# Sinica-SLAM/vae_npvc

Measured on AMD Instinct MI355X. Metric: mel-frames/sec/GPU VQ-VAE train step (80-dim mel, batch=64x256f) at 1/2/4/8 GPUs, higher is better.
Workload: dtype bf16; 1 GPU; vcc20 VQ-VAE (K=512, 80-mel), 64x256 frames per GPU; global_batch=64, seq_len=256, parallelism=dp1

## Files before the change

include/vqx.h:

```cpp
#ifndef VQX_H
#define VQX_H

#include <stdint.h>

#ifdef __cplusplus
extern "C" {
#endif

typedef void* vqx_stream_t;

enum { VQX_F32 = 0, VQX_BF16 = 1 };

enum {
  VQX_PRO_NONE = 0,
  VQX_PRO_LRELU = 1,
  VQX_PRO_RELU = 2,
  VQX_PRO_SCALE_RELU = 3
};

enum {
  VQX_EPI_BIAS = 1 << 0,
  VQX_EPI_ROWBIAS = 1 << 1,
  VQX_EPI_MASK = 1 << 2,
  VQX_EPI_RES = 1 << 3,
  VQX_EPI_GNADD = 1 << 4,
  VQX_EPI_SPLIT = 1 << 5,
  VQX_EPI_OUTF32 = 1 << 6,
  VQX_EPI_ACT = 1 << 7,
  VQX_EPI_ACT2 = 1 << 8,
  VQX_EPI_COLSUM = 1 << 9,
  VQX_EPI_GNSTATS = 1 << 10,
  VQX_EPI_GNBWD = 1 << 11
};
#define VQX_CONV_TILE_ROWS 128

typedef struct vqx_conv_args {
  const void* x;
  const void* w;
  void* y;
  const float* bias;
  const float* rowbias;
  const void* res;
  const void* mask;
  const void* gn_h;
  const float* gn_mean_rstd;
  const float* gn_gamma;
  const float* gn_beta;
  float* out2;
  int64_t n_rows;
  int32_t T;
  int32_t cin, cout, ntaps, pad;
  int32_t ldx, ldy, ldres, ldmask, ldgn, ldo2;
  int32_t dtype;
  int32_t prologue;
  int32_t epilogue;
  int32_t split_col, out2_accumulate;
  float pro_scale, mask_slope, mask_scale;
  void* y2;
  int32_t ldy2, epi_act;
  float* colsum_part;
  float* stat_part;
  int32_t gn_groups, gn_glu;
  const float* gn_stat_tiles;
  float gn_eps;
  int32_t dil;
  int32_t kernel_policy;
  int32_t rowbias_T;
} vqx_conv_args;

#define VQX_POLICY_AUTO 0
#define VQX_POLICY_IM2COL 1
#define VQX_POLICY_TALL256 2
#define VQX_POLICY_TALL512 3
#define VQX_POLICY_TR128 4
#define VQX_POLICY_K1_2PCU 5

int vqx_conv1d_fwd(const vqx_conv_args* a, vqx_stream_t stream);
int vqx_conv1d_dgrad(const vqx_conv_args* a, vqx_stream_t stream);

typedef struct vqx_wgrad_args {
  const void* p;
  const void* q;
  void* slabs;
  int64_t n_rows;
  int32_t T, r_dim, c_dim, ntaps, pad, shift_sign, ldp, ldq;
  int32_t dtype, q_prologue, splits;
  float pro_scale;
  int32_t dil;
  int32_t slab_dtype;
  int32_t kernel_policy;
  float* fixup_dw;
  uint32_t* fixup_counters;
} vqx_wgrad_args;

int vqx_conv1d_wgrad(const vqx_wgrad_args* a, vqx_stream_t stream);
int vqx_wgrad_fixup_ok(int64_t n_rows, int32_t T, int32_t r_dim, int32_t c_dim, int32_t ntaps, int32_t pad, int32_t dil,
                       int32_t dtype, int32_t slab_dtype, int32_t q_prologue, int32_t policy, int32_t* ok);

int vqx_conv1d_dgrad_wgrad(const vqx_conv_args* d, const vqx_wgrad_args* w, int32_t* fused, vqx_stream_t stream);

#define VQX_WN_COLREDUCE 2
#define VQX_WN_RESAMPLE 3
#define VQX_WN_RESAMPLE_T 4
typedef struct vqx_wn_layer {
  const float* v;
  const float* g;
  void* w_packed;
  float* norm;
  float* dv;
  float* dg;
  const void* slabs;
  int32_t kind, cout, cin, k, splits, dtype;
  int32_t stride, pad;
  int32_t slab_dtype;
} vqx_wn_layer;

int vqx_weight_norm_fwd(const vqx_wn_layer* layers_host, const vqx_wn_layer* layers_dev,
                        int32_t n_layers, vqx_stream_t stream);
#define VQX_WNF_NORMS_READY 1
int vqx_weight_norm_fwd_flags(const vqx_wn_layer* layers_host, const vqx_wn_layer* layers_dev,
                              int32_t n_layers, int32_t flags, vqx_stream_t stream);
int vqx_weight_norm_bwd(const vqx_wn_layer* layers_host, const vqx_wn_layer* layers_dev,
                        int32_t n_layers, vqx_stream_t stream);
int vqx_weight_norm_bwd_partials(const vqx_wn_layer* layers_host, int32_t n_layers, int64_t* count);
int vqx_weight_norm_bwd_sq(const vqx_wn_layer* layers_host, const vqx_wn_layer* layers_dev,
                           int32_t n_layers, float* sq_partials, int64_t sq_capacity, vqx_stream_t stream);
int vqx_sq_norm_finish(const float* partials, int64_t n_partials, const float* g, const int64_t* ranges,
                       int32_t n_ranges, float* scratch , float* out, vqx_stream_t stream);
int vqx_sq_norm_finish_adam(const float* partials, int64_t n_partials, const float* g, const int64_t* ranges,
                            int32_t n_ranges, float* scratch, float* out, int64_t* step, double lr0, double gamma,
                            int32_t step_size, double beta1, double beta2, double eps, float* hyper,
                            vqx_stream_t stream);

int vqx_groupnorm_stats(const void* x, int32_t ldx, int32_t dtype, int64_t n_rows, int32_t T,
                        int32_t C, int32_t G, float eps, float* partials ,
                        float* mean_rstd, vqx_stream_t stream);

int vqx_gn_glu_fwd(const void* u, int32_t ldu, void* g, int32_t ldg, int32_t dtype, int64_t n_rows,
                   int32_t T, int32_t C, const float* mean_rstd, const float* gamma, const float* beta,
                   vqx_stream_t stream);

int vqx_gn_glu_fwd_tiles(const void* u, int32_t ldu, void* g, int32_t ldg, int32_t dtype, int64_t n_rows,
                         int32_t T, int32_t C, const float* parts, float eps, float* mean_rstd,
                         const float* gamma, const float* beta, vqx_stream_t stream);

int vqx_gn_lrelu_fwd(const void* h, int32_t ldh, void* g, int32_t ldg, int32_t dtype, int64_t n_rows, int32_t T,
                     int32_t C, const float* mean_rstd, const float* gamma, const float* beta, vqx_stream_t stream);

int vqx_gn_bwd(const void* dy, int32_t lddy, const void* u, int32_t ldu, void* du, int32_t lddu,
               int32_t dtype, int64_t n_rows, int32_t T, int32_t C, int32_t G, int32_t glu,
               const float* mean_rstd, const float* gamma, const float* beta,
               float* partials ,
               int32_t nparts ,
               float* colsum_b , float* dgamma_b , float* dbeta_b ,
               vqx_stream_t stream);

int vqx_gn_finalize_tiles(const float* parts, int64_t n_rows, int32_t T, int32_t C, int32_t G, float eps,
                          float* mean_rstd, vqx_stream_t stream);

int vqx_colsum(const void* x, int32_t ldx, int32_t dtype, int64_t n_rows, int32_t C,
               float* partials , float* out, int32_t accumulate, vqx_stream_t stream);

int vqx_colsum_parts(int64_t n_rows, int32_t C, int32_t dtype, int32_t* nparts);
int vqx_colsum_partials(const void* x, int32_t ldx, int32_t dtype, int64_t n_rows, int32_t C,
                        float* partials , vqx_stream_t stream);

int vqx_nct_to_ntc(const float* x_nct, int32_t B, int32_t C, int32_t T, void* y, int32_t ldy,
                   int32_t dtype, vqx_stream_t stream);
int vqx_ntc_to_nct(const void* y, int32_t ldy, int32_t dtype, int32_t B, int32_t C, int32_t T,
                   float* x_nct, vqx_stream_t stream);

int vqx_logloss_fwd_bwd(const float* x_nct, const float* xhat, int32_t ldxh, int32_t B, int32_t C,
                        int32_t T, float grad_scale, void* dxhat, int32_t lddx, int32_t dtype,
                        float* loss_out, float* partials, vqx_stream_t stream);
int vqx_logloss_fwd_bwd_x(const float* x, const float* xhat, int32_t ldxh, int32_t B, int32_t C, int32_t T,
                          float grad_scale, void* dxhat, int32_t lddx, int32_t dtype, float* loss_out,
                          float* partials, const float* extra_partials, int32_t n_extra, float* extra_out,
                          vqx_stream_t stream);
int vqx_logloss_parts(const float* x, const float* xhat, int32_t ldxh, int32_t B, int32_t C, int32_t T,
                      float grad_scale, void* dxhat, int32_t lddx, int32_t dtype, float* partials, int32_t* n_parts,
                      vqx_stream_t stream);

int vqx_vq_forward(const float* z, int64_t n_rows, int32_t D, const float* E, int32_t K,
                   int64_t* idx, float* zq, void* zq_c, int32_t zq_c_dtype, float* sqerr_out,
                   float* partials, float* bsum, float* bcnt, vqx_stream_t stream);
int vqx_vq_workspace(int64_t n_rows, int32_t K, int32_t D, int32_t with_stats, int64_t* floats);
int vqx_vq_stats(const float* z, int64_t n_rows, int32_t D, const int64_t* idx, int32_t K, float* partials,
                 float* bsum, float* bcnt, vqx_stream_t stream);

int vqx_vq_ema_update(float* emb_sum, float* emb_elem, float* E, const float* bsum,
                      const float* bcnt, const float* rand_rows, int32_t K, int32_t D, float mu,
                      float threshold, float* diag, float* partials, vqx_stream_t stream);
int vqx_vq_ema_update_clear(float* emb_sum, float* emb_elem, float* E, float* bsum, float* bcnt,
                            const float* rand_rows, int32_t K, int32_t D, float mu, float threshold, float* diag,
                            float* partials, vqx_stream_t stream);
typedef struct {
  const float* parts[2];
  int32_t n[2];
  float scale[2];
  float* out[2];
  const float* pub_src;
  int32_t pub_n;
  float* pub_copy;
  void* pub_box;
  int32_t pub_slot, pub_slots, pub_floats;
  uint32_t pub_seq;
  const float* rows_src;
  int32_t rows_ld, n_rows;
  const int32_t* rows_host;
} vqx_step_close;
int vqx_vq_ema_update_close(float* emb_sum, float* emb_elem, float* E, float* bsum, float* bcnt,
                            const float* rand_rows, int32_t K, int32_t D, float mu, float threshold, float* diag,
                            float* partials, const vqx_step_close* close, vqx_stream_t stream);

int vqx_gather_rows(const float* src, int32_t ld_src, const int64_t* rows, int32_t n_out,
                    int32_t D, float* out, vqx_stream_t stream);

int vqx_gather_rows_host(const float* src, int32_t ld_src, const int32_t* rows, int32_t n_out,
                         int32_t D, float* out, vqx_stream_t stream);

int vqx_vq_commit_bwd(const float* z, const float* zq, int64_t count, float scale, void* dz,
                      int32_t dtype, vqx_stream_t stream);
#define VQX_COMMIT_PARTS 256
int vqx_vq_commit_bwd_cs(const float* z, const float* zq, int64_t n_rows, int32_t D, float scale, void* dz,
                         int32_t dtype, float* partials , vqx_stream_t stream);

int vqx_time_gather(const void* x, void* y, int32_t B, int32_t T, int32_t C, const int32_t* src_t,
                    int32_t dtype, vqx_stream_t stream);

int vqx_crop_batch(const float* corpus, int64_t n_rows, int32_t mel, const int64_t* spk_table, int32_t n_utts,
                   const int64_t* row0, const int32_t* len, const int32_t* utt, int32_t B, int32_t T, float* x,
                   int64_t* y, vqx_stream_t stream);

int vqx_embedding_fwd(const float* weight, const int64_t* ids, int32_t B, int32_t D, float* out,
                      vqx_stream_t stream);
int vqx_embedding_bwd(const float* dout, const int64_t* ids, int32_t B, int32_t D, float* dweight,
                      vqx_stream_t stream);
int vqx_embedding_bwd_rows(const float* dout, const int64_t* ids, int32_t B, int32_t D, int32_t n_rows,
                           float* dweight, int32_t accumulate, vqx_stream_t stream);

typedef struct vqx_linear_layer {
  const float* W;
  const float* bias;
  float* out;
  const float* dout;
// ... 10 lines not shown
                      const vqx_linear_layer* cond_table_dev, int32_t n_cond, const float* emb,
                      const int64_t* ids, int32_t B, int32_t I, int32_t O, const float* x_nct, int32_t xB,
                      int32_t C, int32_t T, void* y, int32_t ldy, int32_t y_dtype, vqx_stream_t stream);
int vqx_linear_batched_bwd_ids(const vqx_linear_layer* table_dev, int32_t n, const float* emb,
                               const int64_t* ids, int32_t B, int32_t I, int32_t O, float* dc, float* partials,
                               vqx_stream_t stream);

int vqx_linear_f32(const float* c, const float* W, const float* bias, int32_t B, int32_t I,
                   int32_t O, float* out, vqx_stream_t stream);
int vqx_linear_bwd_f32(const float* dout, const float* c, const float* W, int32_t B, int32_t I,
                       int32_t O, float* dW, float* dc, vqx_stream_t stream);

int vqx_grad_sq_norm(const float* g, int64_t n, float* partials, float* out, vqx_stream_t stream);
int vqx_adam_hyper(int64_t* step, double lr0, double gamma, int32_t step_size, double beta1,
                   double beta2, double eps, float* hyper, vqx_stream_t stream);
int vqx_adam_step(float* p, const float* g, float* m, float* v, int64_t n, const float* hyper,
                  const float* sumsq, float max_norm, vqx_stream_t stream);
int vqx_adam_step_wn(float* p, const float* g, float* m, float* v, int64_t n, const float* hyper,
                     const float* sumsq, float max_norm, const vqx_wn_layer* rows_host,
                     const vqx_wn_layer* rows_dev, int32_t n_layers, const int64_t* segs_host,
                     const int64_t* segs_dev, int32_t n_segs, vqx_stream_t stream);

int vqx_radam_hyper(int64_t* step, double lr0, double gamma, int32_t step_size, double beta1,
                    double beta2, double eps, float* hyper, vqx_stream_t stream);
int vqx_radam_step(float* p, const float* g, float* m, float* v, int64_t n, const float* hyper,
                   const float* sumsq, float max_norm, vqx_stream_t stream);

#define VQX_MULTI_MAX_TENSORS 128
#define VQX_MULTI_CHUNK 4096
int vqx_multi_chunks(const int64_t* numel, int32_t n, int64_t* out);
int vqx_multi_sq_norm(const float* const* grads, const int64_t* numel, int32_t n, float* partials,
                      int64_t n_partials, vqx_stream_t stream);
int vqx_multi_adam_step(float* p, float* m, float* v, int64_t n_flat, const int64_t* offset,
                        const int64_t* numel, const float* const* grads, int32_t n, const float* hyper,
                        const float* sumsq, float max_norm, int32_t kind, vqx_stream_t stream);

int vqx_vq_normalize(const float* z, int64_t n_rows, int32_t D, float* E, int32_t K, float* z_norm,
                     float* z_len, float* emb_norm, float* e_len, float* partials, float* normloss_out,
                     vqx_stream_t stream);
int vqx_vq_perplexity(const float* counts, int32_t K, int64_t n_rows, float* out, vqx_stream_t stream);
int vqx_vq_plain_bwd(const float* z, const float* z_norm, const float* z_len, const float* zq,
                     const void* dzq, const int32_t* src_t, int32_t T, int64_t n_rows, int32_t D,
                     int32_t normalize, float beta, float scale, void* dz, int32_t dtype, const float* bsum,
                     const float* bcnt, const float* emb, const float* e_len, int32_t K, float* dE,
                     vqx_stream_t stream);

int vqx_vq_plain_bwd_g(const float* z, const float* z_norm, const float* z_len, const float* zq, const void* dzq,
                       int32_t T, int64_t n_rows, int32_t D, int32_t normalize, float s_qut, float s_enc,
                       const float* g_qut, const float* g_enc, void* dz, int32_t dtype, const float* bsum,
                       const float* bcnt, const float* emb, const float* e_len, int32_t K, float* dE,
                       vqx_stream_t stream);

int vqx_scale_act_2d(const void* src, int32_t ld_src, int32_t src_dtype, void* dst, int32_t ld_dst,
                     int32_t dst_dtype, int64_t rows, int32_t cols, float scale, int32_t act,
                     vqx_stream_t stream);

int vqx_convert_2d(const void* src, int32_t ld_src, int32_t src_dtype, void* dst, int32_t ld_dst,
                   int32_t dst_dtype, int64_t rows, int32_t cols, vqx_stream_t stream);
int vqx_convert_2d_zero2(const void* src, int32_t ld_src, int32_t src_dtype, void* dst, int32_t ld_dst,
                         int32_t dst_dtype, int64_t rows, int32_t cols, void* zero_dst, int32_t ld_zero,
                         int64_t zero_rows, int32_t zero_cols, vqx_stream_t stream);

int vqx_wgrad_tiles(int64_t n_rows, int32_t T, int32_t r_dim, int32_t c_dim, int32_t ntaps, int32_t pad,
                    int32_t dil, int32_t dtype, int32_t q_prologue, int32_t kernel_policy ,
                    int32_t* tiles);

const char* vqx_last_error(void);

int vqx_probe_enable(int32_t on);
int vqx_probe_select(const int32_t* info5);
int vqx_probe_clear(void);
int vqx_probe_count(int64_t* n);
int vqx_probe_read(int64_t i, int32_t* info5, double* flops, float* ms);

int vqx_stream_create_cu_mask(int32_t reserve_cus, vqx_stream_t* out, int32_t* cus_used);
int vqx_stream_destroy(vqx_stream_t stream);

int vqx_mailbox_create(int32_t slots, int32_t floats, void** host, void** dev);
int vqx_mailbox_destroy(void* host);
int vqx_mailbox_publish(const float* src, int32_t n, float* dev_copy, void* box_dev, int32_t slot, int32_t slots,
                        int32_t floats, uint32_t seq, vqx_stream_t stream);

typedef struct {
  const float* z;
  const float* gst_embs;
  const float *wq, *bq, *wk, *bk, *wv, *bv, *wo, *bo;
  float* style;
  float* ws;
  const float* d_style;
  float* dz;
  float* d_gst_embs;
  float *dwq, *dbq, *dwk, *dbk, *dwv, *dbv, *dwo, *dbo;
  int32_t B, T, R, N, E, F, H, ldz, lddz;
} vqx_gst_args;
int vqx_gst_workspace(int32_t B, int32_t N, int32_t F, int32_t H, int32_t R, int32_t E, int64_t* floats);
int vqx_gst_fwd(const vqx_gst_args* a, vqx_stream_t stream);
int vqx_gst_bwd(const vqx_gst_args* a, vqx_stream_t stream);

typedef struct vqx_hier_level {
  void* z;
  int32_t T_l, C, ld;
} vqx_hier_level;
int vqx_upsample_cat_fwd(const vqx_hier_level* levels, int32_t n_levels, int32_t B, int32_t T, void* out,
                         int32_t ldo, int32_t out_dtype, vqx_stream_t stream);
int vqx_upsample_cat_bwd(const vqx_hier_level* levels, int32_t n_levels, int32_t B, int32_t T, const void* dout,
                         int32_t ldo, int32_t dout_dtype, vqx_stream_t stream);
int vqx_upsample_cat_bwd_to(const vqx_hier_level* levels, int32_t n_levels, int32_t B, int32_t T, const void* dout,
                            int32_t ldo, int32_t dout_dtype, int32_t level_dtype, vqx_stream_t stream);

typedef struct vqx_codes_level {
  const void* z;
  const int64_t* idx;
  int32_t T_l, C, ld;
  int32_t K, normalize;
} vqx_codes_level;
int vqx_codes_upsample_cat(const vqx_codes_level* levels, int32_t n_levels, int32_t B, int32_t T, void* out,
                           int32_t ldo, int32_t out_dtype, vqx_stream_t stream);

int vqx_nct_to_ntc_lrelu_bwd(const float* g_nct, int32_t B, int32_t C, int32_t T, const void* a, int32_t lda,
                             int32_t a_dtype, float slope, void* dst, int32_t lddst, int32_t dst_dtype,
                             vqx_stream_t stream);

int vqx_ntc_to_nct_scale(const float* y, int32_t ldy, int32_t B, int32_t C, int32_t T, const float* g,
                         float* x_nct, vqx_stream_t stream);

int vqx_ntc_to_nct_gather(const void* y, int32_t ldy, int32_t dtype, int32_t B, int32_t C, int32_t T,
                          const int32_t* src_t, float* x_nct, vqx_stream_t stream);
int vqx_nct_to_ntc_keep(const float* g_nct, int32_t B, int32_t C, int32_t T, const int32_t* src_t, void* y,
                        int32_t ldy, int32_t dtype, vqx_stream_t stream);
int vqx_vq_commit_bwd_g(const float* z, const float* zq, int32_t B, int32_t D, int32_t T, float s, const float* g,
                        int32_t nct, float* dz, vqx_stream_t stream);

int vqx_groupnorm_stats_len(const void* x, int32_t ldx, int32_t dtype, int64_t n_rows, int32_t T, int32_t C,
                            int32_t G, const int32_t* len, float eps, float* partials, float* mean_rstd,
                            vqx_stream_t stream);
int vqx_gn_lrelu_fwd_len(const void* h, int32_t ldh, void* g, int32_t ldg, int32_t dtype, int64_t n_rows, int32_t T,
                         int32_t C, const int32_t* len, const float* mean_rstd, const float* gamma, const float* beta,
                         vqx_stream_t stream);
int vqx_gn_glu_fwd_len(const void* u, int32_t ldu, void* g, int32_t ldg, int32_t dtype, int64_t n_rows, int32_t T,
                       int32_t C, const int32_t* len, const float* mean_rstd, const float* gamma, const float* beta,
                       vqx_stream_t stream);
int vqx_mask_tail(void* x, int32_t ldx, int32_t dtype, int64_t n_rows, int32_t T, int32_t C, const int32_t* len,
                  vqx_stream_t stream);
int vqx_codes_upsample_cat_len(const vqx_codes_level* levels, int32_t n_levels, int32_t B, int32_t T,
                               const int32_t* n_len, const int32_t* m_len, void* out, int32_t ldo, int32_t out_dtype,
                               vqx_stream_t stream);
int vqx_segment_mean(const float* z, int32_t ldz, int64_t n_rows, int32_t T, int32_t C, const int32_t* len,
                     float* out, int32_t ldo, vqx_stream_t stream);
int vqx_nct_to_ntc_len(const float* x_nct, int32_t B, int32_t C, int32_t T, const int32_t* len, void* y, int32_t ldy,
                       int32_t dtype, vqx_stream_t stream);
int vqx_ntc_to_nct_len(const void* y, int32_t ldy, int32_t dtype, int32_t B, int32_t C, int32_t T, const int32_t* len,
                       float* x_nct, int32_t T_out, vqx_stream_t stream);

#define VQX_ABI_VERSION 130
int vqx_version(void);

#ifdef __cplusplus
}
#endif
#endif
```

vae_npvc_amd/_lib.py:

```python
import ctypes
import os
from pathlib import Path

import torch

LIB_PATH = Path(__file__).resolve().parent / "lib" / "libvqx.so"
ABI_VERSION = 130

VQX_F32, VQX_BF16 = 0, 1
PRO_NONE, PRO_LRELU, PRO_RELU, PRO_SCALE_RELU = 0, 1, 2, 3
(EPI_BIAS, EPI_ROWBIAS, EPI_MASK, EPI_RES, EPI_GNADD, EPI_SPLIT, EPI_OUTF32, EPI_ACT, EPI_ACT2, EPI_COLSUM, EPI_GNSTATS,
 EPI_GNBWD) = (1 << i for i in range(12))
CONV_TILE_ROWS = 128

c_void_p, c_int32, c_int64, c_float, c_double = (ctypes.c_void_p, ctypes.c_int32, ctypes.c_int64,
                                                 ctypes.c_float, ctypes.c_double)


class ConvArgs(ctypes.Structure):
    _fields_ = [
        ("x", c_void_p), ("w", c_void_p), ("y", c_void_p), ("bias", c_void_p), ("rowbias", c_void_p),
        ("res", c_void_p), ("mask", c_void_p), ("gn_h", c_void_p), ("gn_mean_rstd", c_void_p),
        ("gn_gamma", c_void_p), ("gn_beta", c_void_p), ("out2", c_void_p),
        ("n_rows", c_int64), ("T", c_int32), ("cin", c_int32), ("cout", c_int32), ("ntaps", c_int32),
        ("pad", c_int32), ("ldx", c_int32), ("ldy", c_int32), ("ldres", c_int32), ("ldmask", c_int32),
        ("ldgn", c_int32), ("ldo2", c_int32), ("dtype", c_int32), ("prologue", c_int32),
        ("epilogue", c_int32), ("split_col", c_int32), ("out2_accumulate", c_int32),
        ("pro_scale", c_float), ("mask_slope", c_float), ("mask_scale", c_float),
        ("y2", c_void_p), ("ldy2", c_int32), ("epi_act", c_int32), ("colsum_part", c_void_p),
        ("stat_part", c_void_p), ("gn_groups", c_int32), ("gn_glu", c_int32),
        ("gn_stat_tiles", c_void_p), ("gn_eps", c_float), ("dil", c_int32), ("kernel_policy", c_int32),
        ("rowbias_T", c_int32),
    ]


class WgradArgs(ctypes.Structure):
    _fields_ = [
        ("p", c_void_p), ("q", c_void_p), ("slabs", c_void_p), ("n_rows", c_int64), ("T", c_int32),
        ("r_dim", c_int32), ("c_dim", c_int32), ("ntaps", c_int32), ("pad", c_int32),
        ("shift_sign", c_int32), ("ldp", c_int32), ("ldq", c_int32), ("dtype", c_int32),
        ("q_prologue", c_int32), ("splits", c_int32), ("pro_scale", c_float), ("dil", c_int32),
        ("slab_dtype", c_int32), ("kernel_policy", c_int32), ("fixup_dw", c_void_p), ("fixup_counters", c_void_p),
    ]


class WNLayer(ctypes.Structure):
    _fields_ = [
        ("v", c_void_p), ("g", c_void_p), ("w_packed", c_void_p), ("norm", c_void_p), ("dv", c_void_p),
        ("dg", c_void_p), ("slabs", c_void_p), ("kind", c_int32), ("cout", c_int32), ("cin", c_int32),
        ("k", c_int32), ("splits", c_int32), ("dtype", c_int32), ("stride", c_int32), ("pad", c_int32),
        ("slab_dtype", c_int32),
    ]


class LinearLayer(ctypes.Structure):
    _fields_ = [("W", c_void_p), ("bias", c_void_p), ("out", c_void_p), ("dout", c_void_p), ("dW", c_void_p),
                ("dbias", c_void_p)]


class StepClose(ctypes.Structure):
    _fields_ = [("parts", c_void_p * 2), ("n", c_int32 * 2), ("scale", c_float * 2), ("out", c_void_p * 2),
                ("pub_src", c_void_p), ("pub_n", c_int32), ("pub_copy", c_void_p), ("pub_box", c_void_p),
                ("pub_slot", c_int32), ("pub_slots", c_int32), ("pub_floats", c_int32), ("pub_seq", ctypes.c_uint32),
                ("rows_src", c_void_p), ("rows_ld", c_int32), ("n_rows", c_int32), ("rows_host", c_void_p)]


class GstArgs(ctypes.Structure):
    _fields_ = [
        ("z", c_void_p), ("gst_embs", c_void_p), ("wq", c_void_p), ("bq", c_void_p), ("wk", c_void_p),
        ("bk", c_void_p), ("wv", c_void_p), ("bv", c_void_p), ("wo", c_void_p), ("bo", c_void_p),
        ("style", c_void_p), ("ws", c_void_p), ("d_style", c_void_p), ("dz", c_void_p), ("d_gst_embs", c_void_p),
        ("dwq", c_void_p), ("dbq", c_void_p), ("dwk", c_void_p), ("dbk", c_void_p), ("dwv", c_void_p),
        ("dbv", c_void_p), ("dwo", c_void_p), ("dbo", c_void_p),
        ("B", c_int32), ("T", c_int32), ("R", c_int32), ("N", c_int32), ("E", c_int32), ("F", c_int32),
        ("H", c_int32), ("ldz", c_int32), ("lddz", c_int32),
    ]


class HierLevel(ctypes.Structure):
    _fields_ = [("z", c_void_p), ("T_l", c_int32), ("C", c_int32), ("ld", c_int32)]


class CodesLevel(ctypes.Structure):
    _fields_ = [("z", c_void_p), ("idx", c_void_p), ("T_l", c_int32), ("C", c_int32), ("ld", c_int32),
                ("K", c_int32), ("normalize", c_int32)]


WN_COLREDUCE = 2
WN_RESAMPLE, WN_RESAMPLE_T = 3, 4

_SIGS = {
    "vqx_conv1d_fwd": [ctypes.POINTER(ConvArgs), c_void_p],
    "vqx_conv1d_dgrad": [ctypes.POINTER(ConvArgs), c_void_p],
    "vqx_conv1d_wgrad": [ctypes.POINTER(WgradArgs), c_void_p],
    "vqx_conv1d_dgrad_wgrad": [ctypes.POINTER(ConvArgs), ctypes.POINTER(WgradArgs), ctypes.POINTER(ctypes.c_int32),
                               c_void_p],
    "vqx_weight_norm_fwd": [c_void_p, c_void_p, c_int32, c_void_p],
    "vqx_weight_norm_bwd": [c_void_p, c_void_p, c_int32, c_void_p],
    "vqx_weight_norm_fwd_flags": [c_void_p, c_void_p, c_int32, c_int32, c_void_p],
    "vqx_adam_step_wn": [c_void_p, c_void_p, c_void_p, c_void_p, c_int64, c_void_p, c_void_p, c_float, c_void_p,
                         c_void_p, c_int32, c_void_p, c_void_p, c_int32, c_void_p],
    "vqx_weight_norm_bwd_partials": [c_void_p, c_int32, c_void_p],
    "vqx_weight_norm_bwd_sq": [c_void_p, c_void_p, c_int32, c_void_p, c_int64, c_void_p],
    "vqx_sq_norm_finish": [c_void_p, c_int64, c_void_p, c_void_p, c_int32, c_void_p, c_void_p, c_void_p],
    "vqx_sq_norm_finish_adam": [c_void_p, c_int64, c_void_p, c_void_p, c_int32, c_void_p, c_void_p, c_void_p,
                                c_double, c_double, c_int32, c_double, c_double, c_double, c_void_p, c_void_p],
    "vqx_groupnorm_stats": [c_void_p, c_int32, c_int32, c_int64, c_int32, c_int32, c_int32, c_float, c_void_p,
                            c_void_p, c_void_p],
    "vqx_gn_lrelu_fwd": [c_void_p, c_int32, c_void_p, c_int32, c_int32, c_int64, c_int32, c_int32, c_void_p,
                         c_void_p, c_void_p, c_void_p],
    "vqx_gn_glu_fwd": [c_void_p, c_int32, c_void_p, c_int32, c_int32, c_int64, c_int32, c_int32, c_void_p,
                       c_void_p, c_void_p, c_void_p],
    "vqx_gn_glu_fwd_tiles": [c_void_p, c_int32, c_void_p, c_int32, c_int32, c_int64, c_int32, c_int32, c_void_p,
                             c_float, c_void_p, c_void_p, c_void_p, c_void_p],
    "vqx_gn_bwd": [c_void_p, c_int32, c_void_p, c_int32, c_void_p, c_int32, c_int32, c_int64, c_int32, c_int32,
                   c_int32, c_int32, c_void_p, c_void_p, c_void_p, c_void_p, c_int32, c_void_p, c_void_p, c_void_p,
                   c_void_p],
    "vqx_gn_finalize_tiles": [c_void_p, c_int64, c_int32, c_int32, c_int32, c_float, c_void_p, c_void_p],
    "vqx_colsum": [c_void_p, c_int32, c_int32, c_int64, c_int32, c_void_p, c_void_p, c_int32, c_void_p],
    "vqx_colsum_parts": [c_int64, c_int32, c_int32, c_void_p],
    "vqx_colsum_partials": [c_void_p, c_int32, c_int32, c_int64, c_int32, c_void_p, c_void_p],
    "vqx_nct_to_ntc": [c_void_p, c_int32, c_int32, c_int32, c_void_p, c_int32, c_int32, c_void_p],
    "vqx_ntc_to_nct": [c_void_p, c_int32, c_int32, c_int32, c_int32, c_int32, c_void_p, c_void_p],
    "vqx_logloss_fwd_bwd": [c_void_p, c_void_p, c_int32, c_int32, c_int32, c_int32, c_float, c_void_p, c_int32,
                            c_int32, c_void_p, c_void_p, c_void_p],
    "vqx_logloss_fwd_bwd_x": [c_void_p, c_void_p, c_int32, c_int32, c_int32, c_int32, c_float, c_void_p, c_int32,
                              c_int32, c_void_p, c_void_p, c_void_p, c_int32, c_void_p, c_void_p],
    "vqx_logloss_parts": [c_void_p, c_void_p, c_int32, c_int32, c_int32, c_int32, c_float, c_void_p, c_int32, c_int32,
                          c_void_p, c_void_p, c_void_p],
    "vqx_vq_forward": [c_void_p, c_int64, c_int32, c_void_p, c_int32, c_void_p, c_void_p, c_void_p, c_int32,
                       c_void_p, c_void_p, c_void_p, c_void_p, c_void_p],
    "vqx_vq_workspace": [c_int64, c_int32, c_int32, c_int32, c_void_p],
    "vqx_vq_stats": [c_void_p, c_int64, c_int32, c_void_p, c_int32, c_void_p, c_void_p, c_void_p, c_void_p],
    "vqx_vq_ema_update": [c_void_p, c_void_p, c_void_p, c_void_p, c_void_p, c_void_p, c_int32, c_int32, c_float,
                          c_float, c_void_p, c_void_p, c_void_p],
    "vqx_vq_ema_update_clear": [c_void_p, c_void_p, c_void_p, c_void_p, c_void_p, c_void_p, c_int32, c_int32, c_float,
                                c_float, c_void_p, c_void_p, c_void_p],
    "vqx_vq_ema_update_close": [c_void_p, c_void_p, c_void_p, c_void_p, c_void_p, c_void_p, c_int32, c_int32, c_float,
                                c_float, c_void_p, c_void_p, c_void_p, c_void_p],
    "vqx_gather_rows": [c_void_p, c_int32, c_void_p, c_int32, c_int32, c_void_p, c_void_p],
    "vqx_gather_rows_host": [c_void_p, c_int32, c_void_p, c_int32, c_int32, c_void_p, c_void_p],
    "vqx_vq_commit_bwd": [c_void_p, c_void_p, c_int64, c_float, c_void_p, c_int32, c_void_p],
    "vqx_vq_commit_bwd_cs": [c_void_p, c_void_p, c_int64, c_int32, c_float, c_void_p, c_int32, c_void_p, c_void_p],
    "vqx_time_gather": [c_void_p, c_void_p, c_int32, c_int32, c_int32, c_void_p, c_int32, c_void_p],
    "vqx_crop_batch": [c_void_p, c_int64, c_int32, c_void_p, c_int32, c_void_p, c_void_p, c_void_p, c_int32, c_int32,
                       c_void_p, c_void_p, c_void_p],
    "vqx_embedding_fwd": [c_void_p, c_void_p, c_int32, c_int32, c_void_p, c_void_p],
    "vqx_embedding_bwd": [c_void_p, c_void_p, c_int32, c_int32, c_void_p, c_void_p],
    "vqx_embedding_bwd_rows": [c_void_p, c_void_p, c_int32, c_int32, c_int32, c_void_p, c_int32, c_void_p],
    "vqx_linear_f32": [c_void_p, c_void_p, c_void_p, c_int32, c_int32, c_int32, c_void_p, c_void_p],
    "vqx_linear_bwd_f32": [c_void_p, c_void_p, c_void_p, c_int32, c_int32, c_int32, c_void_p, c_void_p, c_void_p],
    "vqx_grad_sq_norm": [c_void_p, c_int64, c_void_p, c_void_p, c_void_p],
    "vqx_adam_hyper": [c_void_p, c_double, c_double, c_int32, c_double, c_double, c_double, c_void_p, c_void_p],
    "vqx_linear_batched_fwd": [c_void_p, c_int32, c_void_p, c_int32, c_int32, c_int32, c_void_p],
    "vqx_linear_batched_bwd": [c_void_p, c_int32, c_void_p, c_int32, c_int32, c_int32, c_void_p, c_void_p, c_void_p],
    "vqx_linear_batched_fwd_ids": [c_void_p, c_int32, c_void_p, c_void_p, c_int32, c_int32, c_int32, c_void_p],
    "vqx_step_prologue": [c_void_p, c_void_p, c_int32, c_void_p, c_int32, c_void_p, c_void_p, c_int32, c_int32,
                          c_int32, c_void_p, c_int32, c_int32, c_int32, c_void_p, c_int32, c_int32, c_void_p],
    "vqx_linear_batched_bwd_ids": [c_void_p, c_int32, c_void_p, c_void_p, c_int32, c_int32, c_int32, c_void_p,
                                   c_void_p, c_void_p],
    "vqx_wgrad_tiles": [c_int64, c_int32, c_int32, c_int32, c_int32, c_int32, c_int32, c_int32, c_int32, c_int32,
                        ctypes.POINTER(c_int32)],
    "vqx_wgrad_fixup_ok": [c_int64, c_int32, c_int32, c_int32, c_int32, c_int32, c_int32, c_int32, c_int32, c_int32,
                           c_int32, ctypes.POINTER(c_int32)],
    "vqx_vq_normalize": [c_void_p, c_int64, c_int32, c_void_p, c_int32, c_void_p, c_void_p, c_void_p, c_void_p,
                         c_void_p, c_void_p, c_void_p],
    "vqx_vq_perplexity": [c_void_p, c_int32, c_int64, c_void_p, c_void_p],
    "vqx_vq_plain_bwd": [c_void_p, c_void_p, c_void_p, c_void_p, c_void_p, c_void_p, c_int32, c_int64, c_int32,
                         c_int32, c_float, c_float, c_void_p, c_int32, c_void_p, c_void_p, c_void_p, c_void_p,
                         c_int32, c_void_p, c_void_p],
    "vqx_vq_plain_bwd_g": [c_void_p, c_void_p, c_void_p, c_void_p, c_void_p, c_int32, c_int64, c_int32, c_int32,
                           c_float, c_float, c_void_p, c_void_p, c_void_p, c_int32, c_void_p, c_void_p, c_void_p,
                           c_void_p, c_int32, c_void_p, c_void_p],
    "vqx_stream_create_cu_mask": [c_int32, ctypes.POINTER(c_void_p), ctypes.POINTER(c_int32)],
    "vqx_mailbox_create": [c_int32, c_int32, ctypes.POINTER(c_void_p), ctypes.POINTER(c_void_p)],
    "vqx_mailbox_destroy": [c_void_p],
    "vqx_mailbox_publish": [c_void_p, c_int32, c_void_p, c_void_p, c_int32, c_int32, c_int32, ctypes.c_uint32,
                            c_void_p],
    "vqx_stream_destroy": [c_void_p],
    "vqx_probe_enable": [c_int32],
    "vqx_probe_select": [c_void_p],
    "vqx_probe_clear": [],
    "vqx_probe_count": [ctypes.POINTER(c_int64)],
    "vqx_probe_read": [c_int64, ctypes.POINTER(c_int32), ctypes.POINTER(c_double), ctypes.POINTER(c_float)],
    "vqx_scale_act_2d": [c_void_p, c_int32, c_int32, c_void_p, c_int32, c_int32, c_int64, c_int32, c_float, c_int32,
                         c_void_p],
    "vqx_convert_2d": [c_void_p, c_int32, c_int32, c_void_p, c_int32, c_int32, c_int64, c_int32, c_void_p],
    "vqx_convert_2d_zero2": [c_void_p, c_int32, c_int32, c_void_p, c_int32, c_int32, c_int64, c_int32, c_void_p,
                             c_int32, c_int64, c_int32, c_void_p],
    "vqx_adam_step": [c_void_p, c_void_p, c_void_p, c_void_p, c_int64, c_void_p, c_void_p, c_float, c_void_p],
    "vqx_radam_hyper": [c_void_p, c_double, c_double, c_int32, c_double, c_double, c_double, c_void_p, c_void_p],
    "vqx_radam_step": [c_void_p, c_void_p, c_void_p, c_void_p, c_int64, c_void_p, c_void_p, c_float, c_void_p],
    "vqx_multi_chunks": [c_void_p, c_int32, ctypes.POINTER(c_int64)],
    "vqx_multi_sq_norm": [c_void_p, c_void_p, c_int32, c_void_p, c_int64, c_void_p],
    "vqx_multi_adam_step": [c_void_p, c_void_p, c_void_p, c_int64, c_void_p, c_void_p, c_void_p, c_int32, c_void_p,
                            c_void_p, c_float, c_int32, c_void_p],
    "vqx_gst_workspace": [c_int32, c_int32, c_int32, c_int32, c_int32, c_int32, ctypes.POINTER(c_int64)],
    "vqx_gst_fwd": [ctypes.POINTER(GstArgs), c_void_p],
    "vqx_gst_bwd": [ctypes.POINTER(GstArgs), c_void_p],
    "vqx_upsample_cat_fwd": [ctypes.POINTER(HierLevel), c_int32, c_int32, c_int32, c_void_p, c_int32, c_int32,
                             c_void_p],
    "vqx_upsample_cat_bwd": [ctypes.POINTER(HierLevel), c_int32, c_int32, c_int32, c_void_p, c_int32, c_int32,
                             c_void_p],
    "vqx_upsample_cat_bwd_to": [ctypes.POINTER(HierLevel), c_int32, c_int32, c_int32, c_void_p, c_int32, c_int32,
                                c_int32, c_void_p],
    "vqx_codes_upsample_cat": [ctypes.POINTER(CodesLevel), c_int32, c_int32, c_int32, c_void_p, c_int32, c_int32,
                               c_void_p],
    "vqx_groupnorm_stats_len": [c_void_p, c_int32, c_int32, c_int64, c_int32, c_int32, c_int32, c_void_p, c_float,
                                c_void_p, c_void_p, c_void_p],
    "vqx_gn_lrelu_fwd_len": [c_void_p, c_int32, c_void_p, c_int32, c_int32, c_int64, c_int32, c_int32, c_void_p,
                             c_void_p, c_void_p, c_void_p, c_void_p],
    "vqx_gn_glu_fwd_len": [c_void_p, c_int32, c_void_p, c_int32, c_int32, c_int64, c_int32, c_int32, c_void_p,
                           c_void_p, c_void_p, c_void_p, c_void_p],
    "vqx_mask_tail": [c_void_p, c_int32, c_int32, c_int64, c_int32, c_int32, c_void_p, c_void_p],
    "vqx_codes_upsample_cat_len": [ctypes.POINTER(CodesLevel), c_int32, c_int32, c_int32, c_void_p, c_void_p, c_void_p,
                                   c_int32, c_int32, c_void_p],
    "vqx_segment_mean": [c_void_p, c_int32, c_int64, c_int32, c_int32, c_void_p, c_void_p, c_int32, c_void_p],
    "vqx_nct_to_ntc_len": [c_void_p, c_int32, c_int32, c_int32, c_void_p, c_void_p, c_int32, c_int32, c_void_p],
    "vqx_ntc_to_nct_len": [c_void_p, c_int32, c_int32, c_int32, c_int32, c_int32, c_void_p, c_void_p, c_int32,
                           c_void_p],
    "vqx_ntc_to_nct_scale": [c_void_p, c_int32, c_int32, c_int32, c_int32, c_void_p, c_void_p, c_void_p],
    "vqx_nct_to_ntc_lrelu_bwd": [c_void_p, c_int32, c_int32, c_int32, c_void_p, c_int32, c_int32, c_float, c_void_p,
                                 c_int32, c_int32, c_void_p],
    "vqx_ntc_to_nct_gather": [c_void_p, c_int32, c_int32, c_int32, c_int32, c_int32, c_void_p, c_void_p, c_void_p],
    "vqx_nct_to_ntc_keep": [c_void_p, c_int32, c_int32, c_int32, c_void_p, c_void_p, c_int32, c_int32, c_void_p],
    "vqx_vq_commit_bwd_g": [c_void_p, c_void_p, c_int32, c_int32, c_int32, c_float, c_void_p, c_int32, c_void_p,
                            c_void_p],
}
EXPORTS = tuple(_SIGS) + ("vqx_last_error", "vqx_version")


class VqxError(RuntimeError):
    pass


_lib = None


def load(path: os.PathLike = None):
    global _lib
    if _lib is not None:
        return _lib
    path = Path(path or os.environ.get("VQX_LIB") or LIB_PATH)
    if not path.exists():
        raise VqxError(f"libvqx.so not found at {path}; build it with `python -m vae_npvc_amd.csrc.build` "
                       "(the HIP kernels are the only implementation of this path)")
    lib = ctypes.CDLL(str(path), mode=ctypes.RTLD_GLOBAL)
    for name, argtypes in _SIGS.items():
        fn = getattr(lib, name)
        fn.argtypes = argtypes
        fn.restype = ctypes.c_int
    lib.vqx_last_error.restype = ctypes.c_char_p
    lib.vqx_last_error.argtypes = []
    lib.vqx_version.restype = ctypes.c_int
    lib.vqx_version.argtypes = []
    if lib.vqx_version() != ABI_VERSION:
        raise VqxError(f"libvqx ABI {lib.vqx_version()} != expected {ABI_VERSION}; rebuild")
    _lib = lib
    return lib


_post_call = None


def set_post_call(fn):
    global _post_call
    _post_call = fn


def call(name: str, *args):
    lib = load()
    rc = getattr(lib, name)(*args)
    if rc != 0:
        raise VqxError(f"{name} failed ({rc}): {lib.vqx_last_error().decode(errors='replace')}")
    if _post_call is not None:
        _post_call(name)
    return rc


def stream_ptr() -> int:
    return torch.cuda.current_stream().cuda_stream


def ptr(t) -> int:
    return 0 if t is None else t.data_ptr()
```

vae_npvc_amd/csrc/vqx_gemm.hip:

```cpp
#include <hip/hip_ext.h>
#include <stdlib.h>

#include <vector>

#include "vqx_gemm_inst.h"

namespace vqx {

struct ProbeRec {
  hipEvent_t start, stop;
  int info[5];
  double flops;
};
static thread_local bool g_probe_on = false;
static thread_local bool g_probe_sel_on = false;
static thread_local int g_probe_sel[5];
static thread_local std::vector<ProbeRec> g_probe;
static thread_local std::vector<std::pair<hipEvent_t, hipEvent_t>> g_event_pool;
static thread_local size_t g_probe_used = 0;

void gemm_launch(const void* fn, int grid, hipStream_t s, const GemmParams& P, const int info[5], double flops,
                 int block) {
  void* args[] = {(void*)&P};
  gemm_launch_args(fn, grid, s, args, info, flops, block);
}

void gemm_launch_args(const void* fn, int grid, hipStream_t s, void** args, const int info[5], double flops,
                      int block) {
  bool rec = g_probe_on;
  if (rec && g_probe_sel_on)
    for (int i = 0; i < 5; ++i) rec = rec && info[i] == g_probe_sel[i];
  if (!rec) {
    (void)hipLaunchKernel(fn, dim3(grid), dim3(block), args, 0, s);
    return;
  }
  if (g_probe_used == g_event_pool.size()) {
    hipEvent_t a, b;
    if (hipEventCreate(&a) != hipSuccess || hipEventCreate(&b) != hipSuccess) {
      (void)hipLaunchKernel(fn, dim3(grid), dim3(block), args, 0, s);
      return;
    }
    g_event_pool.emplace_back(a, b);
  }
  auto ev = g_event_pool[g_probe_used++];
  ProbeRec r;
  r.start = ev.first;
  r.stop = ev.second;
  for (int i = 0; i < 5; ++i) r.info[i] = info[i];
  r.flops = flops;
  g_probe.push_back(r);
  (void)hipExtLaunchKernel(fn, dim3(grid), dim3(block), args, 0, s, ev.first, ev.second, 0);
}

int cu_count() {
  int dev = 0, n = 0;
  if (hipGetDevice(&dev) != hipSuccess) return 0;
  static thread_local int cached_dev = -1, cached = 0;
  if (dev != cached_dev) {
    if (hipDeviceGetAttribute(&n, hipDeviceAttributeMultiprocessorCount, dev) != hipSuccess) n = 0;
    cached_dev = dev;
    cached = n;
  }
  return cached;
}

bool three_per_cu(int grid, int policy) {
  const int cus = cu_count();
  if (policy == POL_AUTO) return cus > 0 && grid <= 3 * cus;
  return policy == POL_K1_2PCU && cus > 0 && grid > 2 * cus && grid <= 3 * cus;
}

static void launch_mode(GemmParams& P, int mode, int64_t rows, int extra_mult, bool bf16, bool gen, hipStream_t s) {
  P.tiles_m = (int)((rows + 127) / 128);
  const int grid = P.tiles_m * P.tiles_n * extra_mult;
  if (mode == MODE_FWD) launch_mode_dt<MODE_FWD>(P, grid, bf16, gen, s);
  else if (mode == MODE_DGRAD) launch_mode_dt<MODE_DGRAD>(P, grid, bf16, gen, s);
  else launch_mode_dt<MODE_WGRAD>(P, grid, bf16, gen, s);
}

static bool aligned16(const void* p) { return ((uintptr_t)p & 15) == 0; }

static int conv_prepare(const vqx_conv_args* a, int mode, GemmParams& P, bool& gen) {
  if (!a) { set_error("vqx_conv: null args"); return -1; }
  if (a->dtype != VQX_F32 && a->dtype != VQX_BF16) { set_error("vqx_conv: bad dtype %d", a->dtype); return -1; }
  const int epc = a->dtype == VQX_BF16 ? 8 : 4;
  const int es = a->dtype == VQX_BF16 ? 2 : 4;
  const int dil = a->dil > 0 ? a->dil : 1;
  if (a->ntaps < 1 || a->ntaps > 8 || a->pad < 0 || a->pad > (a->ntaps - 1) * dil) { set_error("vqx_conv: ntaps %d / pad %d / dil %d", a->ntaps, a->pad, dil); return -1; }
  if (a->n_rows <= 0 || a->T <= 0 || a->n_rows % a->T) { set_error("vqx_conv: n_rows %lld not a multiple of T %d", (long long)a->n_rows, a->T); return -1; }
  if (a->cin <= 0 || a->cout <= 0 || a->cin % epc || a->ldx % epc || a->cin > a->ldx) { set_error("vqx_conv: cin %d / ldx %d must be multiples of %d", a->cin, a->ldx, epc); return -1; }
  if (a->cout % 8 || a->ldy % 8) { set_error("vqx_conv: cout %d / ldy %d must be multiples of 8", a->cout, a->ldy); return -1; }
  if (mode == MODE_DGRAD && a->cout % epc) { set_error("vqx_conv_dgrad: cout %d must be a multiple of %d", a->cout, epc); return -1; }
  if (!aligned16(a->x) || !aligned16(a->w)) { set_error("vqx_conv: x/w must be 16-byte aligned"); return -1; }
  if (a->prologue < 0 || a->prologue > 3 || (mode == MODE_DGRAD && a->prologue)) { set_error("vqx_conv: bad prologue %d", a->prologue); return -1; }
  const int epi = a->epilogue;
  if ((epi & VQX_EPI_BIAS) && (!a->bias || !aligned16(a->bias))) { set_error("vqx_conv: BIAS needs a 16-B aligned bias"); return -1; }
  if ((epi & VQX_EPI_ROWBIAS) && (!a->rowbias || !aligned16(a->rowbias))) { set_error("vqx_conv: ROWBIAS needs an aligned rowbias"); return -1; }
  if (a->rowbias_T > 1) {
    if (mode != MODE_FWD) { set_error("vqx_conv: rowbias_T %d > 1 is a forward epilogue (not on dgrad)", a->rowbias_T); return -1; }
    if (!(epi & VQX_EPI_ROWBIAS) || a->rowbias_T > a->T) { set_error("vqx_conv: rowbias_T %d needs ROWBIAS and rowbias_T <= T %d", a->rowbias_T, a->T); return -1; }
  } else if (a->rowbias_T < 0) { set_error("vqx_conv: rowbias_T %d < 0", a->rowbias_T); return -1; }
  if ((epi & VQX_EPI_RES) && (!a->res || a->ldres % 8 || !aligned16(a->res))) { set_error("vqx_conv: RES operand"); return -1; }
  if ((epi & VQX_EPI_MASK) && (!a->mask || a->ldmask % 8 || !aligned16(a->mask))) { set_error("vqx_conv: MASK operand"); return -1; }
  if ((epi & VQX_EPI_GNADD) && !(a->gn_h && a->gn_mean_rstd && a->gn_gamma && a->gn_beta && a->ldgn % 8 == 0 && aligned16(a->gn_h) && aligned16(a->gn_gamma) && aligned16(a->gn_beta))) { set_error("vqx_conv: GNADD operands"); return -1; }
  if ((epi & VQX_EPI_SPLIT) && (!a->out2 || a->split_col % 8 || a->ldo2 % 4 || !aligned16(a->out2))) { set_error("vqx_conv: SPLIT operands"); return -1; }
  if ((epi & VQX_EPI_ACT2) && (!a->y2 || a->ldy2 % 8 || !aligned16(a->y2))) { set_error("vqx_conv: ACT2 needs a 16-B aligned y2 with ldy2 %% 8 == 0"); return -1; }
  if ((epi & (VQX_EPI_ACT | VQX_EPI_ACT2)) && a->epi_act != VQX_PRO_LRELU && a->epi_act != VQX_PRO_RELU) { set_error("vqx_conv: epi_act must be LRELU or RELU"); return -1; }
  if (epi & (VQX_EPI_GNSTATS | VQX_EPI_GNBWD)) {
    const int G = a->gn_groups;
    if ((epi & VQX_EPI_GNSTATS) && (epi & VQX_EPI_GNBWD)) { set_error("vqx_conv: GNSTATS and GNBWD are exclusive"); return -1; }
    if (!a->stat_part || a->T % 128 || G < 1 || (epi & VQX_EPI_GNADD)) { set_error("vqx_conv: GN partials need stat_part, T %% 128 == 0, no GNADD"); return -1; }
    if ((epi & VQX_EPI_GNSTATS) && (a->cout % G || (a->cout / G) % 128)) { set_error("vqx_conv: GNSTATS needs cout/G %% 128 == 0"); return -1; }
    if (epi & VQX_EPI_GNBWD) {
      if (!(a->gn_h && a->gn_mean_rstd && a->gn_gamma && aligned16(a->gn_h) && aligned16(a->gn_gamma) && a->ldgn % 8 == 0)) { set_error("vqx_conv: GNBWD operands"); return -1; }
      if (a->gn_glu && (G != 2 || !a->gn_beta || !aligned16(a->gn_beta))) { set_error("vqx_conv: GNBWD glu needs G=2 and beta"); return -1; }
      if (!a->gn_glu && (a->cout % G || (a->cout / G) % 128)) { set_error("vqx_conv: GNBWD needs cout/G %% 128 == 0"); return -1; }
    }
  }
  if ((epi & VQX_EPI_COLSUM) && !a->colsum_part) { set_error("vqx_conv: COLSUM needs colsum_part [ceil(n_rows/128)][cout]"); return -1; }
  if (!a->y || !aligned16(a->y)) { set_error("vqx_conv: y must be non-null and 16-byte aligned"); return -1; }
  if (a->kernel_policy < POL_AUTO || a->kernel_policy > POL_K1_2PCU) { set_error("vqx_conv: kernel_policy %d not in 0..5", a->kernel_policy); return -1; }

  P = GemmParams{};
  P.a = a->x; P.b = a->w;
  P.a_bytes = ((a->n_rows - 1) * (int64_t)a->ldx + a->cin) * es;
  P.n_rows = a->n_rows; P.T = a->T; P.lda = a->ldx;
  P.kcin = a->cin; P.K = a->ntaps * a->cin; P.Mc = (int)a->n_rows; P.Nc = a->cout;
  P.b_bytes = (int64_t)a->ntaps * a->cin * a->cout * es;
  P.ntaps = a->ntaps; P.pad = a->pad; P.sign = 1; P.dil = dil;
  P.cdim = a->cout;
  P.pro = a->prologue; P.pro_scale = a->pro_scale;
  P.tiles_n = (a->cout + kBN - 1) / kBN; P.splits = 1;
  P.y = a->y; P.ldy = a->ldy; P.epi = epi; P.out_f32 = (epi & VQX_EPI_OUTF32) ? 1 : 0;
  P.bias = a->bias; P.rowbias = a->rowbias; P.res = a->res; P.ldres = a->ldres;
  P.mask = a->mask; P.ldmask = a->ldmask; P.mask_slope = a->mask_slope; P.mask_scale = a->mask_scale;
  P.gn_h = a->gn_h; P.ldgn = a->ldgn; P.gn_mr = a->gn_mean_rstd; P.gn_gamma = a->gn_gamma; P.gn_beta = a->gn_beta;
  P.out2 = a->out2; P.ldo2 = a->ldo2; P.split_col = a->split_col; P.out2_acc = a->out2_accumulate;
  P.y2 = a->y2; P.ldy2 = a->ldy2; P.epi_act = a->epi_act;
  P.colsum_part = a->colsum_part;
  P.stat_part = a->stat_part; P.gn_groups = a->gn_groups; P.gn_glu = a->gn_glu;
  P.gn_tiles = a->gn_stat_tiles; P.gn_eps = a->gn_eps;
  P.policy = a->kernel_policy;
  if (a->rowbias_T > 1) {
    const unsigned d = (unsigned)(a->T / a->rowbias_T);
    if ((uint64_t)a->T * d >= (1ull << 32)) { set_error("vqx_conv: rowbias_T: T %d * (T / rowbias_T) must be below 2^32", a->T); return -1; }
    P.rb_T = a->rowbias_T;
    P.rb_magic = d >= 2 ? (unsigned)((1ull << 32) / d) + 1u : 0u;
  }
  if (P.gn_tiles && (mode != MODE_FWD || !(epi & VQX_EPI_GNADD) || a->T % 128 || a->cout % 128 ||
                     a->gn_groups != 1 || !a->gn_mean_rstd)) {
    set_error("vqx_conv: gn_stat_tiles needs FWD with GNADD, G = 1, T %% 128 == 0, cout %% 128 == 0 and gn_mean_rstd");
    return -1;
  }
  if (P.a_bytes > 0x7fffffffLL || P.b_bytes > 0x7fffffffLL) { set_error("vqx_conv: operand larger than 2 GiB"); return -1; }
  gen = (a->cin % (a->dtype == VQX_BF16 ? 64 : 32)) != 0;
  return 0;
}

static int conv_common(const vqx_conv_args* a, int mode, hipStream_t s) {
  GemmParams P;
  bool gen;
  if (conv_prepare(a, mode, P, gen)) return -1;
  launch_mode(P, mode, a->n_rows, 1, a->dtype == VQX_BF16, gen, s);
  return launch_status(mode == MODE_FWD ? "vqx_conv1d_fwd" : "vqx_conv1d_dgrad");
}

static int wgrad_prepare(const vqx_wgrad_args* a, GemmParams& P, bool& gen) {
  if (!a) { set_error("vqx_conv1d_wgrad: null args"); return -1; }
  if (a->dtype != VQX_F32 && a->dtype != VQX_BF16) { set_error("vqx_conv1d_wgrad: bad dtype"); return -1; }
  const int epc = a->dtype == VQX_BF16 ? 8 : 4;
  const int es = a->dtype == VQX_BF16 ? 2 : 4;
  const int dil = a->dil > 0 ? a->dil : 1;
  if (a->ntaps < 1 || a->ntaps > 8 || a->pad < 0 || a->pad > (a->ntaps - 1) * dil) { set_error("vqx_conv1d_wgrad: ntaps %d / pad %d / dil %d", a->ntaps, a->pad, dil); return -1; }
  if (a->n_rows <= 0 || a->T <= 0 || a->n_rows % a->T) { set_error("vqx_conv1d_wgrad: bad n_rows/T"); return -1; }
  if (a->r_dim % epc || a->c_dim % epc || a->ldp % epc || a->ldq % epc || a->c_dim % 8) { set_error("vqx_conv1d_wgrad: dims must be multiples of %d (c_dim of 8)", epc); return -1; }
  if (a->splits < 1) { set_error("vqx_conv1d_wgrad: splits < 1"); return -1; }
  if (!aligned16(a->p) || !aligned16(a->q) || !a->slabs || !aligned16(a->slabs)) { set_error("vqx_conv1d_wgrad: bad pointers"); return -1; }
  if (a->shift_sign != 1 && a->shift_sign != -1) { set_error("vqx_conv1d_wgrad: shift_sign must be +-1"); return -1; }
  if (a->slab_dtype != VQX_F32 && !(a->slab_dtype == VQX_BF16 && a->dtype == VQX_BF16)) { set_error("vqx_conv1d_wgrad: slab_dtype %d (bf16 slabs need bf16 operands)", a->slab_dtype); return -1; }
  if (a->kernel_policy < POL_AUTO || a->kernel_policy > POL_K1_2PCU) { set_error("vqx_conv1d_wgrad: kernel_policy %d not in 0..5", a->kernel_policy); return -1; }
  P = GemmParams{};
  P.a = a->p; P.b = a->q; P.n_rows = a->n_rows; P.T = a->T; P.lda = a->ldp; P.ldb = a->ldq;
  P.a_bytes = ((a->n_rows - 1) * (int64_t)a->ldp + a->r_dim) * es;
  P.b_bytes = ((a->n_rows - 1) * (int64_t)a->ldq + a->c_dim) * es;
  if (P.a_bytes > 0x7fffffffLL || P.b_bytes > 0x7fffffffLL) { set_error("vqx_conv1d_wgrad: operand larger than 2 GiB"); return -1; }
  P.Mc = a->r_dim; P.Nc = a->ntaps * a->c_dim; P.ntaps = a->ntaps; P.pad = a->pad; P.sign = a->shift_sign; P.dil = dil;
  P.cdim = a->c_dim; P.pro = a->q_prologue; P.pro_scale = a->pro_scale;
  P.tiles_n = (P.Nc + kBN - 1) / kBN; P.splits = a->splits;
  int64_t kps = (a->n_rows + a->splits - 1) / a->splits;
  const int kround = a->dtype == VQX_BF16 ? 64 : 32;
  kps = (kps + kround - 1) / kround * kround;
  P.k_per_split = kps;
  P.y = a->slabs;
  P.slab_bf16 = a->slab_dtype == VQX_BF16;
  P.policy = a->kernel_policy;
  const int bkv = a->dtype == VQX_BF16 ? 64 : 32;
  gen = (a->T % bkv) != 0 || (a->n_rows % bkv) != 0;
  if (!gen && wgrad_tr_ok(a->n_rows, a->T, a->c_dim, a->ntaps, a->pad, dil, a->dtype == VQX_BF16, a->q_prologue,
                          a->kernel_policy)) {
    P.tap_reuse = 1;
    P.tiles_n = a->c_dim / 64;
  }
  if (a->fixup_dw) {
    if (!P.tap_reuse || !P.slab_bf16) { set_error("vqx_conv1d_wgrad: fixup_dw needs the 3-tap tap-reuse kernel and bf16 slabs (vqx_wgrad_fixup_ok)"); return -1; }
    if (!aligned16(a->fixup_dw) || !a->fixup_counters) { set_error("vqx_conv1d_wgrad: fixup_dw must be 16-B aligned, fixup_counters non-null"); return -1; }
    if ((int64_t)a->splits * P.Mc * P.Nc * 2 > 0x7fffffffLL) { set_error("vqx_conv1d_wgrad: fixup slabs larger than 2 GiB"); return -1; }
    P.fix_dw = a->fixup_dw;
    P.fix_cnt = a->fixup_counters;
  }
  return 0;
}

}

using namespace vqx;

extern "C" int vqx_conv1d_fwd(const vqx_conv_args* a, vqx_stream_t stream) {
  return conv_common(a, MODE_FWD, (hipStream_t)stream);
}

extern "C" int vqx_conv1d_dgrad(const vqx_conv_args* a, vqx_stream_t stream) {
  return conv_common(a, MODE_DGRAD, (hipStream_t)stream);
}

extern "C" int vqx_conv1d_wgrad(const vqx_wgrad_args* a, vqx_stream_t stream) {
  GemmParams P;
  bool gen;
  if (wgrad_prepare(a, P, gen)) return -1;
  launch_mode(P, MODE_WGRAD, P.Mc, P.splits, a->dtype == VQX_BF16, gen, (hipStream_t)stream);
  return launch_status("vqx_conv1d_wgrad");
}

extern "C" int vqx_conv1d_dgrad_wgrad(const vqx_conv_args* d, const vqx_wgrad_args* w, int32_t* fused,
                                      vqx_stream_t stream) {
  GemmParams PD, PW;
  bool gd, gw;
  if (conv_prepare(d, MODE_DGRAD, PD, gd)) return -1;
  if (wgrad_prepare(w, PW, gw)) return -1;
  hipStream_t s = (hipStream_t)stream;
  const bool bf = d->dtype == VQX_BF16 && w->dtype == VQX_BF16;
  if (bf && !gd && !gw && d->kernel_policy != POL_IM2COL) {
    PD.tiles_m = (int)((d->n_rows + 127) / 128);
    PW.tiles_m = (PW.Mc + 127) / 128;
    if (launch_dual(PD, PD.tiles_m * PD.tiles_n, PW, PW.tiles_m * PW.tiles_n * PW.splits, s)) {
      if (fused) *fused = 1;
      return launch_status("vqx_conv1d_dgrad_wgrad");
    }
  }
  launch_mode(PW, MODE_WGRAD, PW.Mc, PW.splits, w->dtype == VQX_BF16, gw, s);
  launch_mode(PD, MODE_DGRAD, d->n_rows, 1, d->dtype == VQX_BF16, gd, s);
  if (fused) *fused = 0;
  return launch_status("vqx_conv1d_dgrad_wgrad");
}

extern "C" int vqx_wgrad_tiles(int64_t n_rows, int32_t T, int32_t r_dim, int32_t c_dim, int32_t ntaps, int32_t pad,
                               int32_t dil, int32_t dtype, int32_t q_prologue, int32_t policy, int32_t* tiles) {
  if (!tiles || n_rows <= 0 || T <= 0 || r_dim <= 0 || c_dim <= 0 || ntaps < 1 || ntaps > 8 || policy < POL_AUTO ||
      policy > POL_K1_2PCU) {
    set_error("vqx_wgrad_tiles: bad arguments");
    return -1;
  }
  const bool bf16 = dtype == VQX_BF16;
  const int bkv = bf16 ? 64 : 32;
  const bool gen = (T % bkv) != 0 || (n_rows % bkv) != 0;
  const int tm = (r_dim + 127) / 128;
  if (!gen && wgrad_tr_ok(n_rows, T, c_dim, ntaps, pad, dil > 0 ? dil : 1, bf16, q_prologue, policy))
    *tiles = tm * (c_dim / 64);
  else *tiles = tm * ((ntaps * c_dim + kBN - 1) / kBN);
  return 0;
}

extern "C" int vqx_wgrad_fixup_ok(int64_t n_rows, int32_t T, int32_t r_dim, int32_t c_dim, int32_t ntaps, int32_t pad,
                                  int32_t dil, int32_t dtype, int32_t slab_dtype, int32_t q_prologue, int32_t policy,
                                  int32_t* ok) {
  if (!ok || n_rows <= 0 || T <= 0 || r_dim <= 0 || c_dim <= 0 || ntaps < 1 || ntaps > 8) {
    set_error("vqx_wgrad_fixup_ok: bad arguments");
    return -1;
  }
  const bool bf16 = dtype == VQX_BF16;
  const bool gen = (T % 64) != 0 || (n_rows % 64) != 0;
  *ok = (bf16 && slab_dtype == VQX_BF16 && !gen &&
         wgrad_tr_ok(n_rows, T, c_dim, ntaps, pad, dil > 0 ? dil : 1, bf16, q_prologue, policy)) ? 1 : 0;
  return 0;
}

extern "C" int vqx_probe_enable(int32_t on) {
  g_probe_on = on != 0;
  return 0;
}

extern "C" int vqx_probe_select(const int32_t* info5) {
  g_probe_sel_on = info5 != nullptr;
  if (info5)
    for (int i = 0; i < 5; ++i) g_probe_sel[i] = info5[i];
  return 0;
}

extern "C" int vqx_probe_clear(void) {
  g_probe.clear();
  g_probe_used = 0;
  return 0;
}

extern "C" int vqx_probe_count(int64_t* n) {
  if (!n) { set_error("vqx_probe_count: null"); return -1; }
  *n = (int64_t)g_probe.size();
  return 0;
}

extern "C" int vqx_probe_read(int64_t i, int32_t* info5, double* flops, float* ms) {
  if (i < 0 || i >= (int64_t)g_probe.size() || !info5 || !flops || !ms) { set_error("vqx_probe_read: bad index %lld", (long long)i); return -1; }
  const ProbeRec& r = g_probe[i];
  for (int k = 0; k < 5; ++k) info5[k] = r.info[k];
  *flops = r.flops;
  const hipError_t e = hipEventElapsedTime(ms, r.start, r.stop);
  if (e != hipSuccess) { set_error("vqx_probe_read: %s", hipGetErrorString(e)); return -1; }
  return 0;
}
```

vae_npvc_amd/csrc/vqx_gemm_inst.h:

```cpp
#pragma once
#include "vqx_gemm_kernel.h"
#include "vqx_gemm_pp.h"

namespace vqx {

void gemm_launch(const void* fn, int grid, hipStream_t s, const GemmParams& P, const int info[5], double flops,
                 int block = 256);
void gemm_launch_args(const void* fn, int grid, hipStream_t s, void** args, const int info[5], double flops,
                      int block = 256);

bool launch_dual(const GemmParams& PD, int nd, const GemmParams& PW, int nw, hipStream_t s);

enum { POL_AUTO = 0, POL_IM2COL = 1, POL_TALL256 = 2, POL_TALL512 = 3, POL_TR128 = 4, POL_K1_2PCU = 5 };

inline bool tap_reuse_ok(const GemmParams& P, bool bf16, bool gen) {
  return bf16 && P.pro == VQX_PRO_NONE && P.ntaps == 3 && P.pad == 1 && P.dil == 1 && P.kcin % 16 == 0 &&
         (!gen || P.kcin % 32 != 0) && P.K == 3 * P.kcin && P.T % 128 == 0 && P.n_rows % 128 == 0 &&
         P.policy != POL_IM2COL;
}

inline bool wgrad_tr_ok(int64_t n_rows, int T, int c_dim, int ntaps, int pad, int dil, bool bf16, int pro,
                        int policy) {
  return bf16 && pro == VQX_PRO_NONE && ntaps == 3 && pad == 1 && dil == 1 && c_dim % 64 == 0 && T % 64 == 0 &&
         n_rows % 64 == 0 && policy != POL_IM2COL;
}

inline int tr8_segs(const GemmParams& P) {
  if (P.T % 256 || P.kcin % 32) return 0;
  const int tn = (P.Nc + kBN - 1) / kBN;
  if (P.policy == POL_TR128) return 0;
  if (P.policy == POL_TALL256 || P.policy == POL_TALL512) {
    const int segs = P.policy == POL_TALL256 ? 1 : 2;
    return P.n_rows % (256 * segs) == 0 ? segs : 0;
  }
  if (P.n_rows % 512 == 0 && (P.n_rows / 512) * tn >= 256) return 2;
  return 0;
}

#ifndef VQX_TR_FWD_LAB
#define VQX_TR_FWD_LAB 0
#endif

template <int MODE, int EK>
void launch_tr(const GemmParams& P, int grid, hipStream_t s) {
  const double flops = 2.0 * (double)P.n_rows * P.Nc * P.K;
  if constexpr (MODE == MODE_FWD && VQX_TR_FWD_LAB != 0) {
    if (P.policy == POL_AUTO && tr8_segs(P) == 0 && P.T % 256 == 0 && P.n_rows % 256 == 0 && P.kcin % 32 == 0) {
      GemmParams Q = P;
      Q.tiles_m = (int)(P.n_rows / 256);
      const int info8[5] = {VQX_BF16, MODE, 1, 3, EK};
      const void* fn = VQX_TR_FWD_LAB == 1 ? (const void*)conv_tr8_kernel<MODE, EK, 1, 32, 3>
                                           : (const void*)conv_tr8_kernel<MODE, EK, 1, 32, 2>;
      gemm_launch(fn, Q.tiles_m * Q.tiles_n, s, Q, info8, flops, 512);
      return;
    }
  }
  if (int segs = tr8_segs(P)) {
    if (segs == 2 && EK == EK_ALL && P.rb_T) segs = 1;
    GemmParams Q = P;
    Q.tiles_m = (int)(P.n_rows / (256 * segs));
    if (segs == 2) {
      const int infop[5] = {VQX_BF16, MODE, 2, 6, EK};
      gemm_launch((const void*)conv_pp_kernel<MODE, EK, 2, 2>, Q.tiles_m * Q.tiles_n, s, Q, infop, flops, 512);
      return;
    }
    const int info8[5] = {VQX_BF16, MODE, segs, 3, EK};
    gemm_launch((const void*)conv_tr8_kernel<MODE, EK, 1>, Q.tiles_m * Q.tiles_n, s, Q, info8, flops, 512);
    return;
  }
  const int bkc = P.kcin % 32 == 0 ? 32 : 16;
  const int info[5] = {VQX_BF16, MODE, bkc, 2, EK};
  if (bkc == 16) gemm_launch((const void*)conv_tr_kernel<MODE, EK, 16>, grid, s, P, info, flops);
  else gemm_launch((const void*)conv_tr_kernel<MODE, EK, 32>, grid, s, P, info, flops);
}

inline int pick_ek(int epi) {
  for (int ek = EK_NONE; ek < EK_ALL; ++ek)
    if ((epi & ~ek_mask(ek)) == 0) return ek;
  return EK_ALL;
}

template <int MODE>
void dispatch_tr(const GemmParams& P, int grid, hipStream_t s) {
  switch (pick_ek(P.epi)) {
    case EK_NONE: launch_tr<MODE, EK_NONE>(P, grid, s); break;
    case EK_ELEM: launch_tr<MODE, EK_ELEM>(P, grid, s); break;
    case EK_GNADD: launch_tr<MODE, EK_GNADD>(P, grid, s); break;
    case EK_SPLIT: launch_tr<MODE, EK_SPLIT>(P, grid, s); break;
    case EK_COLSUM: launch_tr<MODE, EK_COLSUM>(P, grid, s); break;
    case EK_GNSTATS: launch_tr<MODE, EK_GNSTATS>(P, grid, s); break;
    case EK_GNBWD: launch_tr<MODE, EK_GNBWD>(P, grid, s); break;
    default: launch_tr<MODE, EK_ALL>(P, grid, s); break;
  }
}

int cu_count();
bool three_per_cu(int grid, int policy);

template <typename T, int MODE, int PRO, bool GEN, int EK>
void launch_one(const GemmParams& P, int grid, hipStream_t s) {
  constexpr int BK = sizeof(T) == 2 ? 64 : 32;
  const double flops = MODE == MODE_WGRAD ? 2.0 * (double)P.n_rows * P.Mc * P.Nc
                                          : 2.0 * (double)P.n_rows * P.Nc * P.K;
  if constexpr (sizeof(T) == 2 && !GEN && MODE != MODE_WGRAD && PRO == VQX_PRO_NONE &&
                (EK == EK_NONE || EK == EK_ELEM || EK == EK_SPLIT)) {
    if (P.ntaps == 1 && three_per_cu(grid, P.policy)) {
      const int info3[5] = {VQX_BF16, MODE, P.pro, 4, EK};
      gemm_launch((const void*)conv_gemm3_kernel<T, MODE, PRO, GEN, EK>, grid, s, P, info3, flops);
      return;
    }
  }
  const int info[5] = {sizeof(T) == 2 ? VQX_BF16 : VQX_F32, MODE, P.pro, GEN ? 1 : 0, EK};
  gemm_launch((const void*)conv_gemm_kernel<T, MODE, PRO, GEN, BK, 2, EK>, grid, s, P, info, flops);
}

template <typename T, int MODE, bool GEN, int EK>
void launch_pro(const GemmParams& P, int grid, hipStream_t s) {
  if constexpr (MODE == MODE_DGRAD) {
    launch_one<T, MODE, VQX_PRO_NONE, GEN, EK>(P, grid, s);
  } else {
    switch (P.pro) {
      case VQX_PRO_NONE: launch_one<T, MODE, VQX_PRO_NONE, GEN, EK>(P, grid, s); break;
      case VQX_PRO_LRELU: launch_one<T, MODE, VQX_PRO_LRELU, GEN, EK>(P, grid, s); break;
      case VQX_PRO_RELU: launch_one<T, MODE, VQX_PRO_RELU, GEN, EK>(P, grid, s); break;
      default: launch_one<T, MODE, VQX_PRO_SCALE_RELU, GEN, EK>(P, grid, s); break;
    }
  }
}

template <int MODE>
void launch_mode_dt(const GemmParams& P, int grid, bool bf16, bool gen, hipStream_t s) {
  constexpr int EKW = MODE == MODE_WGRAD ? EK_NONE : EK_ALL;
  if (!bf16) {
    if (gen) launch_pro<float, MODE, true, EKW>(P, grid, s);
    else launch_pro<float, MODE, false, EKW>(P, grid, s);
    return;
  }
  if (gen) {
    if constexpr (MODE != MODE_WGRAD) {
      if (P.pro == VQX_PRO_NONE && tap_reuse_ok(P, bf16, gen)) {
        dispatch_tr<MODE>(P, grid, s);
        return;
      }
    }
    launch_pro<bf16_t, MODE, true, EKW>(P, grid, s);
    return;
  }
  if constexpr (MODE == MODE_WGRAD) {
    if (P.tap_reuse) {
      const double flops = 2.0 * (double)P.n_rows * P.Mc * P.Nc;
      const int info[5] = {VQX_BF16, MODE_WGRAD, 1, 2, EK_NONE};
      gemm_launch((const void*)wgrad_tr_kernel<EK_NONE>, grid, s, P, info, flops);
      return;
    }
    launch_pro<bf16_t, MODE, false, EK_NONE>(P, grid, s);
  } else {
    if (P.pro != VQX_PRO_NONE) {
      launch_pro<bf16_t, MODE, false, EK_ALL>(P, grid, s);
      return;
    }
    if (tap_reuse_ok(P, bf16, gen)) {
      dispatch_tr<MODE>(P, grid, s);
      return;
    }
    switch (pick_ek(P.epi)) {
      case EK_NONE: launch_one<bf16_t, MODE, VQX_PRO_NONE, false, EK_NONE>(P, grid, s); break;
      case EK_ELEM: launch_one<bf16_t, MODE, VQX_PRO_NONE, false, EK_ELEM>(P, grid, s); break;
      case EK_GNADD: launch_one<bf16_t, MODE, VQX_PRO_NONE, false, EK_GNADD>(P, grid, s); break;
      case EK_SPLIT: launch_one<bf16_t, MODE, VQX_PRO_NONE, false, EK_SPLIT>(P, grid, s); break;
      case EK_COLSUM: launch_one<bf16_t, MODE, VQX_PRO_NONE, false, EK_COLSUM>(P, grid, s); break;
      case EK_GNSTATS: launch_one<bf16_t, MODE, VQX_PRO_NONE, false, EK_GNSTATS>(P, grid, s); break;
      case EK_GNBWD: launch_one<bf16_t, MODE, VQX_PRO_NONE, false, EK_GNBWD>(P, grid, s); break;
      default: launch_one<bf16_t, MODE, VQX_PRO_NONE, false, EK_ALL>(P, grid, s); break;
    }
  }
}

}
```

vae_npvc_amd/csrc/vqx_gemm_kernel.h:

```cpp
#pragma once
#include <type_traits>
#include <utility>

#include "vqx_common.h"


namespace vqx {

constexpr int kBN = 128;
constexpr unsigned kOOB = 0x80000000u;
enum { MODE_FWD = 0, MODE_DGRAD = 1, MODE_WGRAD = 2 };

template <typename F, int... I>
__device__ __forceinline__ void static_for_impl(F& f, std::integer_sequence<int, I...>) {
  (f(std::integral_constant<int, I>{}), ...);
}
template <int N, typename F>
__device__ __forceinline__ void static_for(F&& f) {
  static_for_impl(f, std::make_integer_sequence<int, N>{});
}

struct GemmParams {
  const void* a;
  const void* b;
  int64_t a_bytes, b_bytes;
  int64_t n_rows;
  int T, lda, ldb;
  int kcin;
  int K;
  int Mc, Nc;
  int ntaps, pad, sign;
  int dil;
  int cdim;
  int pro;
  float pro_scale;
  int tiles_m, tiles_n, splits;
  int64_t k_per_split;
  void* y;
  int ldy, epi, out_f32;
  const float* bias;
  const float* rowbias;
  const void* res;
  int ldres;
  const void* mask;
  int ldmask;
  float mask_slope, mask_scale;
  const void* gn_h;
  int ldgn;
  const float* gn_mr;
  const float* gn_gamma;
  const float* gn_beta;
  float* out2;
  int ldo2, split_col, out2_acc;
  void* y2;
  int ldy2, epi_act;
  float* colsum_part;
  float* stat_part;
  int gn_groups, gn_glu;
  int tap_reuse;
  int slab_bf16;
  const float* gn_tiles;
  float gn_eps;
  int policy;
  float* fix_dw;
  unsigned* fix_cnt;
  int rb_T;
  unsigned rb_magic;
};

template <typename T> struct Cfg;
template <> struct Cfg<bf16_t> { static constexpr int EPC = 8, MNCPR = 16; };
template <> struct Cfg<float> { static constexpr int EPC = 4, MNCPR = 32; };

__device__ __forceinline__ float apply_pro(float v, int pro, float s) {
  if (pro == VQX_PRO_LRELU) return v > 0.f ? v : 0.2f * v;
  if (pro == VQX_PRO_RELU) return v > 0.f ? v : 0.f;
  if (pro == VQX_PRO_SCALE_RELU) { v = v * s; return v > 0.f ? v : 0.f; }
  return v;
}

template <typename T, int PRO>
__device__ __forceinline__ uint4 pro_chunk(uint4 u, float s) {
  if constexpr (PRO == VQX_PRO_NONE) {
    return u;
  } else if constexpr (sizeof(T) == 2) {
    unsigned w[4] = {u.x, u.y, u.z, u.w};
#pragma unroll
    for (int i = 0; i < 4; ++i) {
      float lo = __uint_as_float(w[i] << 16), hi = __uint_as_float(w[i] & 0xffff0000u);
      lo = apply_pro(lo, PRO, s);
      hi = apply_pro(hi, PRO, s);
      w[i] = pack_bf16x2(lo, hi);
    }
    return make_uint4(w[0], w[1], w[2], w[3]);
  } else {
    float f[4] = {__uint_as_float(u.x), __uint_as_float(u.y), __uint_as_float(u.z), __uint_as_float(u.w)};
#pragma unroll
    for (int i = 0; i < 4; ++i) f[i] = apply_pro(f[i], PRO, s);
    return make_uint4(__float_as_uint(f[0]), __float_as_uint(f[1]), __float_as_uint(f[2]), __float_as_uint(f[3]));
  }
}

__device__ __forceinline__ int tap_of(int k, int c, int nt) {
  if (nt <= 3) return (k >= c) + (k >= 2 * c);
  int j = 0;
#pragma unroll
  for (int t = 1; t < 8; ++t) j += (t < nt && k >= t * c) ? 1 : 0;
  return j;
}

__device__ __forceinline__ __amdgpu_buffer_rsrc_t rsrc_at(const void* base, int64_t shift_bytes, int64_t total_bytes) {
  int64_t rec = total_bytes - shift_bytes;
  if (rec < 0) rec = 0;
  if (rec > 0x7fffffff) rec = 0x7fffffff;
  return __builtin_amdgcn_make_buffer_rsrc((void*)((const char*)base + shift_bytes), (short)0, (int)rec, 0x00020000);
}

__device__ __forceinline__ uint4 bload(__amdgpu_buffer_rsrc_t r, unsigned off) {
  typedef unsigned int u32x4 __attribute__((ext_vector_type(4)));
  const u32x4 v = __builtin_amdgcn_raw_buffer_load_b128(r, (int)off, 0, 0);
  return make_uint4(v[0], v[1], v[2], v[3]);
}

template <int KCH>
__device__ __forceinline__ int kswz(int row) {
  if constexpr (KCH == 8) return (row >> 1) & 7;
  else return (row >> 2) & 3;
}
template <int KCH>
__device__ __forceinline__ int kmaj_off(int row, int ch) { return row * (16 * KCH) + 16 * (ch ^ kswz<KCH>(row)); }
__device__ __forceinline__ int mn_swz(int row) { return ((row & 3) << 2) | ((row >> 2) & 3); }
template <typename T>
__device__ __forceinline__ int mnmaj_off(int row, int ch) {
  if constexpr (sizeof(T) == 2) return row * 256 + 16 * (ch ^ mn_swz(row));
  else return row * 512 + 16 * ch;
}

template <typename T>
__device__ __forceinline__ void ld8(const void* p, int64_t i, float* f) {
  if constexpr (sizeof(T) == 2) {
    const uint4 u = *(const uint4*)((const bf16_t*)p + i);
    const unsigned w[4] = {u.x, u.y, u.z, u.w};
#pragma unroll
    for (int k = 0; k < 4; ++k) {
      f[2 * k] = __uint_as_float(w[k] << 16);
      f[2 * k + 1] = __uint_as_float(w[k] & 0xffff0000u);
    }
  } else {
    const f32x4_t a = *(const f32x4_t*)((const float*)p + i);
    const f32x4_t b = *(const f32x4_t*)((const float*)p + i + 4);
#pragma unroll
    for (int k = 0; k < 4; ++k) { f[k] = a[k]; f[4 + k] = b[k]; }
  }
}
template <typename T>
__device__ __forceinline__ void st8(void* p, int64_t i, const float* f) {
  if constexpr (sizeof(T) == 2) {
    uint4 u;
    u.x = pack_bf16x2(f[0], f[1]);
    u.y = pack_bf16x2(f[2], f[3]);
    u.z = pack_bf16x2(f[4], f[5]);
    u.w = pack_bf16x2(f[6], f[7]);
    *(uint4*)((bf16_t*)p + i) = u;
  } else {
    const f32x4_t a = {f[0], f[1], f[2], f[3]}, b = {f[4], f[5], f[6], f[7]};
    *(f32x4_t*)((float*)p + i) = a;
    *(f32x4_t*)((float*)p + i + 4) = b;
  }
}

template <typename T, bool NT = true>
__device__ __forceinline__ void st8_nt(void* p, int64_t i, const float* f) {
  if constexpr (!NT) {
    st8<T>(p, i, f);
    return;
  }
  typedef unsigned u32x4v __attribute__((ext_vector_type(4)));
  if constexpr (sizeof(T) == 2) {
    const u32x4v u = {pack_bf16x2(f[0], f[1]),
                      pack_bf16x2(f[2], f[3]),
                      pack_bf16x2(f[4], f[5]),
                      pack_bf16x2(f[6], f[7])};
    __builtin_nontemporal_store(u, (u32x4v*)((bf16_t*)p + i));
  } else {
    const f32x4_t a = {f[0], f[1], f[2], f[3]}, b = {f[4], f[5], f[6], f[7]};
    __builtin_nontemporal_store(a, (f32x4_t*)((float*)p + i));
    __builtin_nontemporal_store(b, (f32x4_t*)((float*)p + i + 4));
  }
}

enum {
  EK_NONE = 0,
  EK_ELEM = 1,
  EK_GNADD = 2,
  EK_SPLIT = 3,
  EK_COLSUM = 4,
  EK_GNSTATS = 5,
  EK_GNBWD = 6,
  EK_ALL = 7
};
constexpr int kEpiElem = VQX_EPI_BIAS | VQX_EPI_ROWBIAS | VQX_EPI_MASK | VQX_EPI_RES | VQX_EPI_ACT | VQX_EPI_ACT2 |
                         VQX_EPI_OUTF32;
__host__ __device__ constexpr int ek_mask(int ek) {
  return ek == EK_NONE ? VQX_EPI_OUTF32
       : ek == EK_ELEM ? kEpiElem
       : ek == EK_GNADD ? kEpiElem | VQX_EPI_GNADD
       : ek == EK_SPLIT ? kEpiElem | VQX_EPI_SPLIT
       : ek == EK_COLSUM ? kEpiElem | VQX_EPI_COLSUM
       : ek == EK_GNSTATS ? kEpiElem | VQX_EPI_GNSTATS
       : ek == EK_GNBWD ? kEpiElem | VQX_EPI_COLSUM | VQX_EPI_GNBWD
       : ~0;
}

enum { EPR_NONE = 0, EPR_GNH, EPR_GNH2, EPR_MASK, EPR_RES };
typedef unsigned u32x4e_t __attribute__((ext_vector_type(4)));
struct EpiRows {
  u32x4e_t r0[8], r1[8];
  int k0, k1;
};

template <int EK, int I0 = 0, int NR = 8>
__device__ __forceinline__ void epi_prefetch(const GemmParams& P, int m0, int n0, int tid, EpiRows& R) {
  constexpr int EM = ek_mask(EK);
  const int epi = P.epi & EM;
  const int er = tid >> 4, col = n0 + (tid & 15) * 8;
  const bool to_out2 = (epi & VQX_EPI_SPLIT) && col >= P.split_col;
  const bool g = epi & (VQX_EPI_GNADD | VQX_EPI_GNBWD), g2 = (epi & VQX_EPI_GNBWD) && P.gn_glu;
  const bool mk = (epi & VQX_EPI_MASK) && !to_out2, rs = (epi & VQX_EPI_RES) && !to_out2;
  const int k0 = g ? EPR_GNH : mk ? EPR_MASK : rs ? EPR_RES : EPR_NONE;
  const int k1 = g ? (g2 ? EPR_GNH2 : mk ? EPR_MASK : rs ? EPR_RES : EPR_NONE) : (mk && rs) ? EPR_RES : EPR_NONE;
  R.k0 = k0;
  R.k1 = k1;
  auto addr = [&](int k, int64_t row) -> const u32x4e_t* {
    const bf16_t* b = k == EPR_MASK ? (const bf16_t*)P.mask + row * P.ldmask
                    : k == EPR_RES  ? (const bf16_t*)P.res + row * P.ldres
                                    : (const bf16_t*)P.gn_h + row * P.ldgn + (k == EPR_GNH2 ? P.Nc : 0);
    return (const u32x4e_t*)(b + col);
  };
  static_for<NR>([&](auto i_c) __attribute__((always_inline)) {
    constexpr int i = I0 + decltype(i_c)::value;
    const int64_t row = (int64_t)m0 + (i >> 2) * 64 + (i & 3) * 16 + er;
    const bool ok = row < P.n_rows && col < P.Nc;
    const u32x4e_t z = {0u, 0u, 0u, 0u};
    R.r0[i] = (ok && k0 != EPR_NONE) ? *addr(k0, row) : z;
    R.r1[i] = (ok && k1 != EPR_NONE) ? *addr(k1, row) : z;
  });
}

__device__ __forceinline__ void unpack8(u32x4e_t u, float* f) {
  const unsigned w[4] = {u[0], u[1], u[2], u[3]};
#pragma unroll
  for (int k = 0; k < 4; ++k) {
    f[2 * k] = __uint_as_float(w[k] << 16);
    f[2 * k + 1] = __uint_as_float(w[k] & 0xffff0000u);
  }
}

struct EpiOps {
  u32x4e_t p0, p1;
  int k0, k1;
};
template <int I, bool PRE>
__device__ __forceinline__ EpiOps epi_ops(const EpiRows* R) {
  EpiOps o = {{0u, 0u, 0u, 0u}, {0u, 0u, 0u, 0u}, EPR_NONE, EPR_NONE};
  if constexpr (PRE) {
    o.p0 = R->r0[I];
    o.p1 = R->r1[I];
    o.k0 = R->k0;
    o.k1 = R->k1;
  }
  return o;
}

struct EpiVec {
  float b[8], ga[8], be[8], gb[8], bb[8];
  float mr[4];
  bool mr_ok;
};
template <int EMASK>
__device__ __forceinline__ void epi_vec_load(const GemmParams& P, int col, EpiVec& V, int m0 = 0) {
  const int epi = P.epi & EMASK;
  V.mr_ok = false;
  if ((epi & VQX_EPI_GNBWD) && P.T % 128 == 0 && (P.gn_glu || P.gn_groups == 1)) {
    const int b = m0 / P.T, n = P.gn_glu ? 4 : 2;
#pragma unroll
    for (int i = 0; i < 4; ++i) V.mr[i] = i < n ? P.gn_mr[b * n + i] : 0.f;
    V.mr_ok = true;
  }
  if (col >= P.Nc) return;
  if (epi & VQX_EPI_BIAS) ld8<float>(P.bias, col, V.b);
  if (epi & (VQX_EPI_GNADD | VQX_EPI_GNBWD)) {
    ld8<float>(P.gn_gamma, col, V.ga);
    if (!(epi & VQX_EPI_GNBWD) || P.gn_glu) ld8<float>(P.gn_beta, col, V.be);
    if ((epi & VQX_EPI_GNBWD) && P.gn_glu) {
      ld8<float>(P.gn_gamma, col + P.Nc, V.gb);
      ld8<float>(P.gn_beta, col + P.Nc, V.bb);
    }
  }
}
template <bool PRE>
__device__ __forceinline__ void vec8(const float (&pre)[8], const float* p, int64_t i, float* f) {
  if constexpr (PRE) {
#pragma unroll
    for (int e = 0; e < 8; ++e) f[e] = pre[e];
  } else {
    ld8<float>(p, i, f);
  }
}

template <typename T>
__device__ __forceinline__ void row_op(const EpiOps& o, int role, const void* base, int64_t off, float* t) {
  if constexpr (sizeof(T) == 2) {
    if (o.k0 == role) { unpack8(o.p0, t); return; }
    if (o.k1 == role) { unpack8(o.p1, t); return; }
  }
  ld8<T>(base, off, t);
}

template <typename T, int EMASK, bool PRE = false, bool SEG = false>
__device__ __forceinline__ void epilogue8(const GemmParams& P, int64_t row, int col, float* v, const float* gmr,
                                          const EpiOps& o, const EpiVec& V) {
  const int epi = P.epi & EMASK;
  const int bidx = (epi & (VQX_EPI_ROWBIAS | VQX_EPI_GNADD)) ? (int)row / P.T : 0;
  float t[8];
  if (epi & VQX_EPI_BIAS) {
    vec8<PRE>(V.b, P.bias, col, t);
#pragma unroll
    for (int e = 0; e < 8; ++e) v[e] += t[e];
  }
  if (epi & VQX_EPI_ROWBIAS) {
    int ridx = bidx;
    if constexpr (SEG) {
      if (__builtin_expect(P.rb_T != 0, 0)) {
        const unsigned t_in = (unsigned)((int)row - bidx * P.T);
        const int seg = (int)(P.rb_magic ? __umulhi(t_in, P.rb_magic) : t_in);
        ridx = bidx * P.rb_T + (seg < P.rb_T ? seg : P.rb_T - 1);
      }
    }
    ld8<float>(P.rowbias, (int64_t)ridx * P.Nc + col, t);
#pragma unroll
    for (int e = 0; e < 8; ++e) v[e] += t[e];
  }
  if (epi & VQX_EPI_MASK) {
    row_op<T>(o, EPR_MASK, P.mask, row * P.ldmask + col, t);
#pragma unroll
    for (int e = 0; e < 8; ++e) v[e] *= (t[e] > 0.f ? 1.f : P.mask_slope) * P.mask_scale;
  }
  if ((epi & VQX_EPI_SPLIT) && col >= P.split_col) {
    float* o2 = P.out2 + row * P.ldo2 + (col - P.split_col);
    if (P.out2_acc) {
      ld8<float>(o2, 0, t);
#pragma unroll
      for (int e = 0; e < 8; ++e) v[e] += t[e];
    }
    st8<float>(o2, 0, v);
#pragma unroll
    for (int e = 0; e < 8; ++e) v[e] = 0.f;
    return;
  }
  if (epi & VQX_EPI_RES) {
    row_op<T>(o, EPR_RES, P.res, row * P.ldres + col, t);
#pragma unroll
    for (int e = 0; e < 8; ++e) v[e] += t[e];
  }
  if (epi & VQX_EPI_GNADD) {
    float ga[8], be[8];
    row_op<T>(o, EPR_GNH, P.gn_h, row * P.ldgn + col, t);
    vec8<PRE>(V.ga, P.gn_gamma, col, ga);
    vec8<PRE>(V.be, P.gn_beta, col, be);
    const float mean = gmr[2 * bidx], rstd = gmr[2 * bidx + 1];
#pragma unroll
    for (int e = 0; e < 8; ++e) v[e] += (t[e] - mean) * rstd * ga[e] + be[e];
  }
  if (epi & (VQX_EPI_ACT | VQX_EPI_ACT2)) {
#pragma unroll
    for (int e = 0; e < 8; ++e) t[e] = apply_pro(v[e], P.epi_act, 1.f);
    if (epi & VQX_EPI_ACT2) {
      st8<T>(P.y2, row * P.ldy2 + col, t);
    } else {
#pragma unroll
      for (int e = 0; e < 8; ++e) v[e] = t[e];
    }
  }
  if (P.out_f32) st8_nt<float, false>(P.y, row * P.ldy + col, v);
  else st8_nt<T, false>(P.y, row * P.ldy + col, v);
}

template <typename T, bool PRE = false>
__device__ __forceinline__ void gnbwd8(const GemmParams& P, int64_t row, int col, const float* dy, float* s,
                                       const EpiOps& o, const EpiVec& V) {
  const int b = (int)row / P.T;
  float ua[8], ga[8];
  row_op<T>(o, EPR_GNH, P.gn_h, row * P.ldgn + col, ua);
  vec8<PRE>(V.ga, P.gn_gamma, col, ga);
  const bool mr_pre = PRE && V.mr_ok;
  if (!P.gn_glu) {
    const int grp = P.gn_groups == 1 ? 0 : col / (P.Nc / P.gn_groups);
    const float m = mr_pre ? V.mr[0] : P.gn_mr[(b * P.gn_groups + grp) * 2];
    const float r = mr_pre ? V.mr[1] : P.gn_mr[(b * P.gn_groups + grp) * 2 + 1];
#pragma unroll
    for (int e = 0; e < 8; ++e) {
      const float g = ga[e] * dy[e];
      s[0] += g;
      s[1] = fmaf(g, (ua[e] - m) * r, s[1]);
    }
    return;
  }
  const int half = P.Nc;
  float ub[8], gb[8], ba[8], bb[8];
  row_op<T>(o, EPR_GNH2, P.gn_h, row * P.ldgn + col + half, ub);
  vec8<PRE>(V.gb, P.gn_gamma, col + half, gb);
  vec8<PRE>(V.be, P.gn_beta, col, ba);
  vec8<PRE>(V.bb, P.gn_beta, col + half, bb);
  const float ma = mr_pre ? V.mr[0] : P.gn_mr[b * 4], ra = mr_pre ? V.mr[1] : P.gn_mr[b * 4 + 1];
  const float mb = mr_pre ? V.mr[2] : P.gn_mr[b * 4 + 2], rb = mr_pre ? V.mr[3] : P.gn_mr[b * 4 + 3];
#pragma unroll
  for (int e = 0; e < 8; ++e) {
    const float xa = (ua[e] - ma) * ra, xb = (ub[e] - mb) * rb;
    const float ta = ftanh<sizeof(T) == 2>(xa * ga[e] + ba[e]);
    const float sb = fsigmoid<sizeof(T) == 2>(xb * gb[e] + bb[e]);
    const float dga = ga[e] * (dy[e] * sb * (1.f - ta * ta));
    const float dgb = gb[e] * (dy[e] * ta * (sb * (1.f - sb)));
    s[0] += dga;
    s[1] = fmaf(dga, xa, s[1]);
    s[2] += dgb;
    s[3] = fmaf(dgb, xb, s[3]);
  }
}

template <int PRO>
__device__ __forceinline__ bf16x8_t pro_frag(bf16x8_t f, float s) {
  if constexpr (PRO == VQX_PRO_NONE) {
    return f;
  } else {
    uint4 u = __builtin_bit_cast(uint4, f);
    u = pro_chunk<bf16_t, PRO>(u, s);
    return __builtin_bit_cast(bf16x8_t, u);
  }
}
template <int PRO>
__device__ __forceinline__ f32x4_t pro_frag(f32x4_t f, float s) {
  if constexpr (PRO == VQX_PRO_NONE) {
    return f;
  } else {
#pragma unroll
    for (int i = 0; i < 4; ++i) f[i] = apply_pro(f[i], PRO, s);
    return f;
  }
}


__device__ __forceinline__ void dma16(__amdgpu_buffer_rsrc_t r, char* lds, unsigned off) {
  const unsigned la = __builtin_amdgcn_readfirstlane((unsigned)(uintptr_t)(VQX_LDS(void)*)lds);
  asm volatile("s_mov_b32 m0, %0\n\ts_nop 0\n\tbuffer_load_dwordx4 %1, %2, 0 offen lds" ::"s"(la), "v"(off), "s"(r)
               : "memory", "m0");
}

__device__ __forceinline__ void wait_vm(int n) {
  switch (n) {
    case 0: asm volatile("s_waitcnt vmcnt(0)" ::: "memory"); break;
    case 1: asm volatile("s_waitcnt vmcnt(1)" ::: "memory"); break;
    case 2: asm volatile("s_waitcnt vmcnt(2)" ::: "memory"); break;
    case 3: asm volatile("s_waitcnt vmcnt(3)" ::: "memory"); break;
    case 4: asm volatile("s_waitcnt vmcnt(4)" ::: "memory"); break;
    case 5: asm volatile("s_waitcnt vmcnt(5)" ::: "memory"); break;
    case 6: asm volatile("s_waitcnt vmcnt(6)" ::: "memory"); break;
    case 7: asm volatile("s_waitcnt vmcnt(7)" ::: "memory"); break;
    case 8: asm volatile("s_waitcnt vmcnt(8)" ::: "memory"); break;
    case 10: asm volatile("s_waitcnt vmcnt(10)" ::: "memory"); break;
    case 12: asm volatile("s_waitcnt vmcnt(12)" ::: "memory"); break;
    case 16: asm volatile("s_waitcnt vmcnt(16)" ::: "memory"); break;
    default: asm volatile("s_waitcnt vmcnt(0)" ::: "memory"); break;
  }
}

template <typename T, int MODE, int EK, bool PRE = false, bool PREVEC = PRE, bool SEGOK = true>
__device__ __forceinline__ void tile_epilogue(const GemmParams& P, f32x16_t (&acc)[2][2], char* smem, int m0, int n0,
                                              int tn, int split, const float* gmr, int tid,
                                              const EpiRows* R = nullptr) {
  constexpr int EMASK = ek_mask(EK);
  constexpr int SUB = 1;
  const int lane = tid & 63;
  const int wid = __builtin_amdgcn_readfirstlane(tid >> 6);
  const int wm = wid >> 1, wn = wid & 1;
  const int r32 = lane & 31, h = lane >> 5;
  constexpr int EP_LD = kBN + 4;
  constexpr int EROWS = 16 * SUB;
  float* ep = (float*)smem;
  float* csr = (float*)smem;
  const int er = tid >> 4, ec = (tid & 15) * 8;
  float cs[8] = {0.f, 0.f, 0.f, 0.f, 0.f, 0.f, 0.f, 0.f};
  float mn = 0.f, mm = 0.f, mq = 0.f;
  float gs[4] = {0.f, 0.f, 0.f, 0.f};
  EpiVec V;
  if constexpr (PREVEC && MODE != MODE_WGRAD) epi_vec_load<EMASK>(P, n0 + ec, V, m0);
  __syncthreads();
  static_for<2 * SUB>([&](auto slab_c) __attribute__((always_inline)) {
    constexpr int slab = decltype(slab_c)::value;
    if (wm == slab) {
#pragma unroll
      for (int mi = 0; mi < 2; ++mi)
#pragma unroll
        for (int ni = 0; ni < 2; ++ni)
#pragma unroll
          for (int gq = 0; gq < 4; ++gq) {
            const f32x4_t v = {acc[mi][ni][4 * gq], acc[mi][ni][4 * gq + 1], acc[mi][ni][4 * gq + 2],
                               acc[mi][ni][4 * gq + 3]};
            *(f32x4_t*)(ep + (mi * 32 + r32) * EP_LD + wn * 64 + ni * 32 + 8 * gq + 4 * h) = v;
          }
    }
    __syncthreads();
    static_for<64 / EROWS>([&](auto pass_c) __attribute__((always_inline)) {
      constexpr int pass = decltype(pass_c)::value;
      const int lr = pass * EROWS + er;
      const f32x4_t lo = *(const f32x4_t*)(ep + lr * EP_LD + ec);
      const f32x4_t hi = *(const f32x4_t*)(ep + lr * EP_LD + ec + 4);
      float v[8] = {lo[0], lo[1], lo[2], lo[3], hi[0], hi[1], hi[2], hi[3]};
      const int64_t row = (int64_t)m0 + slab * 64 + lr;
      const int col = n0 + ec;
      if constexpr (MODE == MODE_WGRAD) {
        if (row < P.Mc && col < P.Nc) {
          const int64_t at = (int64_t)split * P.Mc * P.Nc + row * P.Nc + col;
          if (sizeof(T) == 2 && P.slab_bf16) st8<bf16_t>(P.y, at, v);
          else st8_nt<float, false>((float*)P.y + at, 0, v);
        }
      } else {
        if (row < P.n_rows && col < P.Nc) {
          const EpiOps o = epi_ops<slab * 4 + pass, PRE>(R);
          epilogue8<T, EMASK, PREVEC, MODE == MODE_FWD && SEGOK>(P, row, col, v, gmr, o, V);
#pragma unroll
          for (int e = 0; e < 8; ++e) cs[e] += v[e];
          if (P.epi & EMASK & VQX_EPI_GNSTATS) {
            float m8 = 0.f;
#pragma unroll
            for (int e = 0; e < 8; ++e) m8 += v[e];
            m8 *= 0.125f;
            float q8 = 0.f;
#pragma unroll
            for (int e = 0; e < 8; ++e) q8 = fmaf(v[e] - m8, v[e] - m8, q8);
            moments_merge(mn, mm, mq, 8.f, m8, q8);
          }
          if (P.epi & EMASK & VQX_EPI_GNBWD) gnbwd8<T, PREVEC>(P, row, col, v, gs, o, V);
        }
      }
    });
    __syncthreads();
    if constexpr (MODE != MODE_WGRAD) {
      if ((P.epi & EMASK & (VQX_EPI_GNSTATS | VQX_EPI_GNBWD)) && (slab & 1)) {
        const int64_t grp_row = (int64_t)m0 + (slab >> 1) * 128;
        float* out = P.stat_part + ((grp_row / 128) * P.tiles_n + tn) * 4;
        if (P.epi & EMASK & VQX_EPI_GNSTATS) {
#pragma unroll
          for (int o = 1; o < 64; o <<= 1) {
            const float n2 = __shfl_xor(mn, o, 64), m2 = __shfl_xor(mm, o, 64), q2 = __shfl_xor(mq, o, 64);
            if ((lane & o) == 0) moments_merge(mn, mm, mq, n2, m2, q2);
            else { float a = n2, b = m2, c = q2; moments_merge(a, b, c, mn, mm, mq); mn = a; mm = b; mq = c; }
          }
          if (lane == 0) { csr[3 * wid] = mn; csr[3 * wid + 1] = mm; csr[3 * wid + 2] = mq; }
          __syncthreads();
          if (tid == 0 && grp_row < P.n_rows) {
            float a = csr[0], b = csr[1], c = csr[2];
            for (int w = 1; w < 4 * SUB; ++w) moments_merge(a, b, c, csr[3 * w], csr[3 * w + 1], csr[3 * w + 2]);
            out[0] = a; out[1] = b; out[2] = c; out[3] = 0.f;
          }
          mn = mm = mq = 0.f;
        } else {
#pragma unroll
          for (int k = 0; k < 4; ++k) {
            float x = wave_sum(gs[k]);
            if (lane == 0) csr[4 * wid + k] = x;
            gs[k] = 0.f;
          }
          __syncthreads();
          if (tid < 4 && grp_row < P.n_rows) {
            float x = 0.f;
            for (int w = 0; w < 4 * SUB; ++w) x += csr[4 * w + tid];
            out[tid] = x;
          }
        }
        __syncthreads();
      }
      if ((P.epi & EMASK & VQX_EPI_COLSUM) && (slab & 1)) {
#pragma unroll
        for (int e = 0; e < 8; ++e) {
          csr[er * kBN + ec + e] = cs[e];
          cs[e] = 0.f;
        }
        __syncthreads();
        const int64_t grp_row = (int64_t)m0 + (slab >> 1) * 128;
        if (tid < kBN && n0 + tid < P.Nc && grp_row < P.n_rows) {
          float t = 0.f;
#pragma unroll
          for (int r = 0; r < EROWS; ++r) t += csr[r * kBN + tid];
          P.colsum_part[(grp_row / 128) * P.Nc + n0 + tid] = t;
        }
        __syncthreads();
      }
    }
  });
}

constexpr int kEpiBytes = 64 * (kBN + 4) * 4;
template <typename T, int BK, int NST>
__host__ __device__ constexpr int conv_gemm_smem() {
  return NST * 2 * 128 * BK * (int)sizeof(T) > kEpiBytes ? NST * 2 * 128 * BK * (int)sizeof(T) : kEpiBytes;
}

template <typename T, int MODE, int PRO, bool GEN, int BK, int NST, int EK>
__device__ __forceinline__ void conv_gemm_body(const GemmParams& P, int bid, int nwg, char* smem) {
  using C = Cfg<T>;
  constexpr int EPC = C::EPC, CPR = C::MNCPR, ES = sizeof(T);
  constexpr int BM = 128;
  constexpr int RB = BK * ES;
  constexpr int KCH = RB / 16;
  constexpr int OP_BYTES = 128 * BK * ES;
  constexpr int PW = OP_BYTES / 1024 / 4;
  constexpr int A_BYTES = OP_BYTES, STAGE = 2 * OP_BYTES;
  constexpr int NP = 2 * PW;
  static_assert(conv_gemm_smem<T, BK, NST>() >= kEpiBytes, "epilogue staging needs 33 KiB of LDS");
  static_assert(BK % (16 / ES * 2) == 0 || ES == 4, "BK");
  static_assert(conv_gemm_smem<T, BK, NST>() >= NST * STAGE, "LDS");

  const int tid = threadIdx.x, lane = tid & 63;
  const int wid = __builtin_amdgcn_readfirstlane(tid >> 6);
  const int wm = wid >> 1, wn = wid & 1;
  const int lin = xcd_remap(bid, nwg);
  const int tiles_mn = P.tiles_m * P.tiles_n;
  const int split = lin / tiles_mn;
  const int tmn = lin - split * tiles_mn;
  const int tm = tmn / P.tiles_n, tn = tmn - tm * P.tiles_n;
  const int m0 = tm * BM, n0 = tn * kBN;

  __shared__ float gmr_s[2];
  const float* gmr = P.gn_mr;
  if constexpr ((ek_mask(EK) & VQX_EPI_GNADD) != 0 && MODE == MODE_FWD) {
    if (P.gn_tiles != nullptr && (P.epi & VQX_EPI_GNADD)) {
      const int b0 = m0 / P.T;
      if (tid == 0) {
        const int rg = P.T / 128, ntn = P.Nc / 128;
        double n = 0.0, mean = 0.0, m2 = 0.0;
        for (int r = 0; r < rg; ++r)
          for (int t = 0; t < ntn; ++t) {
            const float* o = P.gn_tiles + ((int64_t)(b0 * rg + r) * ntn + t) * 4;
            const double nb = o[0];
            if (nb == 0.0) continue;
            const double d = (double)o[1] - mean;
            const double nn = n + nb;
            mean += d * nb / nn;
            m2 += (double)o[2] + d * d * n * nb / nn;
            n = nn;
          }
        const float var = n > 0.0 ? (float)(m2 / n) : 0.f;
        gmr_s[0] = (float)mean;
        gmr_s[1] = 1.0f / sqrtf(var + P.gn_eps);
        if (tn == 0 && m0 % P.T == 0) {
          ((float*)P.gn_mr)[2 * b0] = gmr_s[0];
          ((float*)P.gn_mr)[2 * b0 + 1] = gmr_s[1];
        }
      }
      gmr = gmr_s - 2 * b0;
    }
  }

  int64_t kbeg = 0, kend;
  if constexpr (MODE == MODE_WGRAD) {
    kbeg = (int64_t)split * P.k_per_split;
    kend = kbeg + P.k_per_split;
    if (kend > P.n_rows) kend = P.n_rows;
  } else {
    kend = P.K;
  }
  const int nk = (kend > kbeg) ? (int)((kend - kbeg + BK - 1) / BK) : 0;

  unsigned aoff[PW], boff[PW];
  int amask[PW];
// ... 887 lines not shown
```

vae_npvc_amd/engine/step.py:

```python
import bisect
import math
from dataclasses import dataclass, field

import numpy as np
import torch

from .. import _lib as L
from .. import ops

F32 = torch.float32
KIND_CONV, KIND_CONVT, KIND_DOWN, KIND_UP = 0, 1, 3, 4


@dataclass(eq=False)
class ConvLayer:
    mod: object
    name: str
    kind: int
    cin: int
    cout: int
    k: int
    pad: int
    dil: int = 1
    scale: int = 1
    wp: torch.Tensor = None
    norm: torch.Tensor = None
    slab: torch.Tensor = None
    splits: int = 1
    fix_dw: torch.Tensor = None
    fix_cnt: torch.Tensor = None
    btile: torch.Tensor = None

    @property
    def rows(self):
        return self.cin if self.kind in (KIND_CONVT, KIND_UP) else self.cout

    @property
    def cols(self):
        if self.kind == KIND_DOWN:
            return 3 * self.scale * self.cin
        if self.kind == KIND_UP:
            return 3 * self.scale * self.cout
        return (self.cout if self.kind == KIND_CONVT else self.cin) * self.k


@dataclass
class EncBlock:
    key: tuple
    convs: list
    gns: list
    skip: ConvLayer


@dataclass
class EncStage:
    conv: ConvLayer
    scale: int
    C: int
    blocks: list = field(default_factory=list)
    L: int = 1


@dataclass
class DecBlock:
    key: tuple
    gidx: int
    conv_in: ConvLayer
    gn: object
    cond: ConvLayer
    rs: ConvLayer


@dataclass
class DecStage:
    conv: ConvLayer
    scale: int
    C: int
    blocks: list = field(default_factory=list)


def _tm(N):
    return (N + L.CONV_TILE_ROWS - 1) // L.CONV_TILE_ROWS


def _wn_block_bytes(e):
    if e["kind"] == L.WN_COLREDUCE:
        return e["cin"] * 32 * 4
    rows_cout = e["kind"] in (0, L.WN_RESAMPLE)
    other = e["cin"] if rows_cout else e["cout"]
    cols = 3 * e.get("stride", 1) * other if e["kind"] in (L.WN_RESAMPLE, L.WN_RESAMPLE_T) else other * e["k"]
    sl = e.get("slabs")
    es = sl.element_size() if sl is not None else 4
    b = cols * (e.get("splits", 1) * es + 8)
    wave_rows = e["kind"] == 0 and e["k"] == 1 and e["cin"] <= 256 and (e["cin"] // 4) * e.get("splits", 1) <= 256
    return 4 * b if wave_rows else b


@dataclass
class EngineOptions:
    fuse_gn: bool = True
    enc_gn_finalize: bool = False
    side_stream: bool = False
    wgrad_wgs: int = 256
    wgrad_wgs_1x1: int = 256
    wgrad_wgs_solo: int = 512
    wgrad_min_k: int = 512
    slab_f32: bool = False
    wn_bwd_batch: bool = True
    wn_bwd_ddp_groups: int = 5
    wn_bwd_sort: bool = True
    lazy_stats: bool = True
    fuse_grad_norm: bool = True
    fuse_adam_wn: bool = True
    kernel_policy: int = 0
    debug_checks: bool = False
    wgrad_fixup: bool = False
    early_stats: bool = True
    fused_prologue: bool = True
    fused_close: bool = True
    bwd_streams: bool = True
    wn_bwd_split: bool = False
    enc_bwd_early: bool = True
    side_priority: int = 0
    vq_stats_side: bool = False
    bwd_streams_ddp: bool = True


class _Stage:
    """Per-stage activation buffers of a Workspace."""


class Workspace:

    def __init__(self, eng, B, T, train=True):
        d, cd, dev = eng.dims, eng.cd, eng.device
        self.B, self.T, self.N = B, T, B * T
        e = lambda *s, dt=cd: eng._empty(*s, dtype=dt)
        Z, S, Fo, mel, K = d["Z"], d["S"], d["F"], d["mel"], d["K"]
        fuse_opt = eng.opt.fuse_gn
        self.x = e(self.N, mel)
        self.enc = []
        Tc = T
        for st in eng.enc_stages:
            if Tc % st.scale:
                raise ValueError(f"utterance length {Tc} is not a multiple of the down-sampling scale {st.scale}")
            Tc //= st.scale
            sw = _Stage()
            sw.T, sw.N, sw.C = Tc, B * Tc, st.C
            N, C, nb = sw.N, sw.C, len(st.blocks)
            sw.c = [e(N, C) for _ in range(nb + 1)]
            sw.a = [e(N, C) for _ in range(nb + 1)]
            sw.h = [[e(N, C) for _ in range(st.L)] for _ in range(nb)]
            sw.g = [[e(N, C) for _ in range(st.L - 1)] for _ in range(nb)]
            sw.mr = [[e(B, 2, dt=F32) for _ in range(st.L)] for _ in range(nb)]
            sw.fuse = Tc % 128 == 0 and C % 128 == 0 and fuse_opt
            if train:
                sw.cs = [e(_tm(N), C, dt=F32) for _ in range(nb + 1)]
            self.enc.append(sw)
        self.Tz, self.Nz = Tc, B * Tc
        Nz = self.Nz
        self.z = e(Nz, Z, dt=F32)
        self.idx = torch.empty(Nz, device=dev, dtype=torch.int64)
        self.zq = e(Nz, Z, dt=F32)
        self.zq_c = e(Nz, Z)
        self.zq_j = e(Nz, Z) if d["jitter_p"] > 0 else None
        self.src_t = torch.empty(Tc, device=dev, dtype=torch.int32)
        self.jittered = False
        if eng.plain:
            self.z_norm = e(Nz, Z, dt=F32)
            self.z_len = e(Nz, dt=F32)
            self.embn = e(K, Z, dt=F32)
            self.e_len = e(K, dt=F32)
            self.pv_part = e(Nz // 4 + 8, dt=F32)
        self.vq_part = e(ops.vq_workspace(Nz, K, train or eng.plain, Z), dt=F32)
        self.ema = e(K * Z + K + K * Z, dt=F32)
        self.bsum = self.ema[: K * Z].view(K, Z)
        self.bcnt = self.ema[K * Z: K * Z + K]
        self.rand_rows = self.ema[K * Z + K:].view(K, Z)
        self.ema_part = eng._zeros(ops.ema_workspace(K, Z), dtype=F32)
        self.yemb = e(B, d["ydim"], dt=F32)
        self.dec = []
        Td = Tc
        for st in eng.dec_stages:
            Td *= st.scale
            sw = _Stage()
            sw.T, sw.N, sw.C = Td, B * Td, st.C
            N, C, nb = sw.N, sw.C, len(st.blocks)
            sw.xs = [e(N, C) for _ in range(nb + 1)]
            sw.u = [e(N, 2 * C) for _ in range(nb)]
            sw.g = [e(N, C) for _ in range(nb)]
            sw.mr = [e(B, 4, dt=F32) for _ in range(nb)]
            sw.condbias = [e(B, 2 * C, dt=F32) for _ in range(nb)]
            sw.fuse = Td % 128 == 0 and C % 128 == 0 and fuse_opt
            if train:
                sw.dr = [e(N, C + S) for _ in range(2)] if nb else None
                sw.dx = e(N, C) if not nb else None
                sw.cs = [e(_tm(N), C, dt=F32) for _ in range(nb + 1)]
                sw.cs[-1].zero_()
                sw.cs_all = [e(B, 2 * C, dt=F32) for _ in range(nb)]
            self.dec.append(sw)
        if Td != T:
            raise ValueError(f"decoder output length {Td} != input length {T} (resampling scales do not cancel)")
        if eng.n_dec_blocks:
            Ts = self.dec[eng.skip_stage].T
            if any(sw.T != Ts for sw, st in zip(self.dec, eng.dec_stages) if st.blocks):
                raise ValueError("the decoder sums the skip outputs of all blocks: they must share one frame rate")
        self.Nskip = B * T
        self.skip32 = e(self.Nskip, S, dt=F32)
        self.a_skip = e(self.Nskip, S)
        self.f1 = e(self.Nskip, S)
        self.xhat = e(self.N, Fo, dt=F32)
        self.xhat_nct = e(B, Fo, T, dt=F32)
        self.stats = eng._zeros(8, dtype=F32)
        Cmax = max([sw.C for sw in self.enc] + [2 * sw.C for sw in self.dec] + [1])
        Nmax = max([sw.N for sw in self.enc] + [sw.N for sw in self.dec] + [self.N])
        self.gst = e(max(1, Nmax // 128) * ((Cmax + 127) // 128) * 4, dt=F32)
        self.loss_part = e(1024, dt=F32)
        self.gn_part = e(B * 2 * 8 * 3, dt=F32)
        if not train:
            return
        NCe = max([sw.N * sw.C for sw in self.enc] + [1])
        if eng.fin2_pad is not None:
            self.dxhat_pad = eng._zeros(self.N, eng.fin2_pad[0], dtype=cd)
            self.dxhat = self.dxhat_pad[:, :Fo]
        else:
            self.dxhat = self.dxhat_pad = e(self.N, Fo)
        self.df1 = e(self.Nskip, S)
        NCd = max([sw.N * sw.C for sw in self.dec] + [1])
        self.dg_flat = e(NCd)
        self.du_flat = e(2 * NCd)
        self.gnb_part = e(max(B * 64 * 2, max(1, Nmax // 128) * ((Cmax + 127) // 128) * 4), dt=F32)
        self.gnb_part_enc = e(self.gnb_part.numel(), dt=F32)
        Lmax = max([st.L for st in eng.enc_stages] + [1])
        self.colsum_b = [e(B * 2 * Cmax, dt=F32) for _ in range(Lmax)]
        self.dgam_b = [e(B * 2 * Cmax, dt=F32) for _ in range(Lmax)]
        self.dbet_b = [e(B * 2 * Cmax, dt=F32) for _ in range(Lmax)]
        self.blk_parts = {}
        if eng.opt.wn_bwd_batch:
            for si, st in enumerate(eng.enc_stages):
                for j in range(len(st.blocks)):
                    self.blk_parts[("enc", si, j)] = {k: [e(B * self.enc[si].C, dt=F32) for _ in range(st.L)]
                                                      for k in ("colsum_b", "dgam_b", "dbet_b")}
            for si, st in enumerate(eng.dec_stages):
                for j in range(len(st.blocks)):
                    self.blk_parts[("dec", si, j)] = {k: [e(B * 2 * self.dec[si].C, dt=F32)]
                                                      for k in ("dgam_b", "dbet_b")}
        self.dz = e(Nz, Z)
        self.dzq = e(Nz, Z) if eng.plain else None
        self.dc_flat = [e(NCe) for _ in range(2)]
        self.dh_flat = e(NCe)
        self.dy_flat = e(NCe)
        self.tmp_flat = e(NCe)
        self.dyemb = e(B, d["ydim"], dt=F32)
        self.cs_part = e(64 * max(Cmax, S + Cmax, mel, 1024), dt=F32)
        self.cs_part_enc = e(self.cs_part.numel(), dt=F32)
        self.cs_skip = e(_tm(self.Nskip), S, dt=F32)
        self.cs_f1 = e(_tm(self.Nskip), S, dt=F32)
        self.cs_eo = eng._zeros(ops.COMMIT_PARTS, Z, dtype=F32)
        self.cs_f2 = e(ops.colsum_parts(self.N, Fo, cd), Fo, dt=F32)
        self.lin_part = e(max(len(g) * ((O + 63) // 64) for O, g in eng.cond_groups.items()) * B * d["ydim"]
                          if eng.cond_groups else 1, dt=F32)
        eng._build_bwd_tables(self)

    @staticmethod
    def view(flat, N, C):
        return flat[: N * C].view(N, C)


class VQVAEEngine:
    def __init__(self, model, device, compute_dtype="fp32", options=None):
        self.m = model
        self.opt = options if options is not None else EngineOptions()
        self.device = torch.device(device)
        self.cd = torch.bfloat16 if compute_dtype in ("bf16", "bfloat16") else F32
        self.dt = ops.dt_code(self.cd)
        L.load()
        self._guards = None
        if self.opt.debug_checks:
# ... 471 lines not shown
            s = Lr.scale
            ops.conv_wgrad(dy, x.view(-1, s * Lr.cin), Lr.slab, T=T, r_dim=Lr.cout, c_dim=s * Lr.cin, ntaps=3, pad=1,
                           shift_sign=1, splits=Lr.splits, policy=pol)
        else:
            s = Lr.scale
            ops.conv_wgrad(x, dy.view(-1, s * Lr.cout), Lr.slab, T=T // s, r_dim=Lr.cin, c_dim=s * Lr.cout, ntaps=3,
                           pad=1, shift_sign=1, splits=Lr.splits, policy=pol)

    def wgrad_dgrad(self, Lr, dy, x, dx, T, **kw):
        if Lr.kind not in (KIND_CONV, KIND_CONVT):
            self.wgrad(Lr, dy, x, T)
            self.dgrad(Lr, dy, dx, T, **kw)
            return
        pol = self.opt.kernel_policy
        dkw = dict(T=T, cin=Lr.cout, cout=Lr.cin, ntaps=Lr.k, pad=(Lr.k - 1) * Lr.dil - Lr.pad, dil=Lr.dil, policy=pol,
                   **kw)
        wkw = dict(T=T, ntaps=Lr.k, pad=Lr.pad, dil=Lr.dil, splits=Lr.splits, policy=pol)
        if id(Lr) in self._fix_now:
            wkw.update(fixup_dw=Lr.fix_dw, fixup_counters=Lr.fix_cnt)
        if Lr.kind == KIND_CONV:
            ops.conv_dgrad_wgrad(dy, Lr.wp, dx, dkw, dy, x, Lr.slab, dict(wkw, r_dim=Lr.cout, c_dim=Lr.cin, shift_sign=1))
        else:
            ops.conv_dgrad_wgrad(dy, Lr.wp, dx, dkw, x, dy, Lr.slab, dict(wkw, r_dim=Lr.cin, c_dim=Lr.cout, shift_sign=-1))

    def bias_grad(self, part, dy, zero_tail=False):
        n = ops.colsum_parts(dy.shape[0], dy.shape[1], dy.dtype)
        ops.colsum_partials(dy, part[:n])
        if zero_tail and n < part.shape[0]:
            ops.zero_(part[n:])

    def pack_weights(self):
        plan = self._adam_wn
        if plan is not None and self._packed_version == self._param_version():
            if plan[2] is not None:
                ops.weight_norm_fwd(plan[2], flags=plan[3])
            if self._guards is not None:
                self._check_packed()
        else:
            ops.weight_norm_fwd(self.wn_fwd_table)
        self._up_bias()

    def _up_bias(self):
        for st in self.dec_stages:
            if st.conv.kind == KIND_UP:
                s = st.conv.scale
                ops.convert_2d(st.conv.mod.bias.detach().view(1, -1).expand(s, -1), st.conv.btile.view(s, -1))

    def _side_stream(self):
        if self._side is None:
            self._side = torch.cuda.Stream(device=self.device, priority=self.opt.side_priority)
        return self._side

    def _join(self):
        if self._side is not None and self._side_pending:
            torch.cuda.current_stream().wait_stream(self._side)
            self._side_pending = False

    def _fork(self):
        side = self._side_stream()
        side.wait_stream(torch.cuda.current_stream())
        self._side_pending = True
        return side

    def _cond_ids(self, w, ids):
        emb = self.m.embeds._embedding.weight
        return (getattr(w, "cond_tables", None) is not None and bool(self.cond_groups) and ids.dtype == torch.int64
                and all(ops.linear_ids_ok(w.B, blocks[0].cond.cin, O, emb) for O, blocks in self.cond_groups.items()))

    def embed_and_cond(self, w, y):
        ids = y.reshape(-1)
        emb = self.m.embeds._embedding.weight
        w.cond_ids_mode = self._cond_ids(w, ids)
        if w.cond_ids_mode:
            for O, blocks in self.cond_groups.items():
                ops.linear_batched_fwd_ids(w.cond_tables[O], emb, ids, w.B, blocks[0].cond.cin, O)
            return
        ops.embedding_fwd(emb, ids, w.yemb)
        tabs = getattr(w, "cond_tables", None)
        for O, blocks in self.cond_groups.items():
            if tabs is not None:
                ops.linear_batched_fwd(tabs[O], w.yemb, w.B, blocks[0].cond.cin, O)
            else:
                for b in blocks:
                    ops.linear_f32(w.yemb, b.cond.wp, b.cond.mod.bias, w.dec[b.key[1]].condbias[b.key[2]])

    def _fused_prologue(self, w, x):
        plan = self._adam_wn
        if (not self.opt.fused_prologue or self._side_on or plan is None
                or self._packed_version != self._param_version() or not x.is_contiguous()):
            return False
        if plan[2] is not None and (len(plan[2][0]) > 256 or not (plan[3] & ops.WNF_NORMS_READY
                                                                  or all(e.kind != 1 for e in plan[2][0]))):
            return False
        cond = None
        if len(self.cond_groups) == 1 and self._cond_ids(w, w.y_dev):
            (O, blocks), = self.cond_groups.items()
            w.cond_ids_mode = True
            cond = (w.cond_tables[O], self.m.embeds._embedding.weight, w.y_dev, w.B, blocks[0].cond.cin, O)
        else:
            self.embed_and_cond(w, w.y_dev)
        ops.step_prologue(plan[2], cond, x, w.x)
        self._up_bias()
        if self._guards is not None:
            self._check_packed()
        self.n_fused_prologue = getattr(self, "n_fused_prologue", 0) + 1
        return True

    def encoder_fwd(self, w, x_nct, transposed=False, lens=None):
        if lens is not None:
            ops.nct_to_ntc_len(x_nct, lens, w.x)
        elif not transposed:
            ops.nct_to_ntc(x_nct, w.x)
        inp, T_in = w.x, w.T
        for si, st in enumerate(self.enc_stages):
            sw = w.enc[si]
            T = sw.T
            self.fwd(st.conv, inp, sw.c[0], T_in, bias=st.conv.mod.bias, act=L.PRO_LRELU, y2=sw.a[0])
            if lens is not None:
                lens = [n // st.scale for n in lens]
                ops.mask_tail(sw.a[0], T, lens)
            for j, b in enumerate(st.blocks):
                src = sw.a[j]
                gkw = {}
                for l, (Lr, gn) in enumerate(zip(b.convs, b.gns)):
                    h, mr = sw.h[j][l], sw.mr[j][l]
                    last = l == st.L - 1
                    if lens is not None:
                        self.fwd(Lr, src, h, T, bias=Lr.mod.bias)
                        ops.groupnorm_stats_len(h, T, 1, lens, w.gn_part, mr)
                    elif sw.fuse:
                        self.fwd(Lr, src, h, T, bias=Lr.mod.bias, gn_stats=w.gst, gn_groups=1)
                        if last and not self._enc_gn_separate:
                            gkw = dict(gn_tiles=w.gst)
                        else:
                            ops.gn_finalize_tiles(w.gst, sw.N, T, sw.C, 1, mr)
                    else:
                        self.fwd(Lr, src, h, T, bias=Lr.mod.bias)
                        ops.groupnorm_stats(h, T, 1, w.gn_part, mr)
                    if not last:
                        if lens is not None:
                            ops.gn_lrelu_fwd_len(h, sw.g[j][l], T, lens, mr, gn.weight, gn.bias)
                        else:
                            ops.gn_lrelu_fwd(h, sw.g[j][l], T, mr, gn.weight, gn.bias)
                        src = sw.g[j][l]
                gn = b.gns[-1]
                self.fwd(b.skip, sw.c[j], sw.c[j + 1], T, bias=b.skip.mod.bias, gn_h=sw.h[j][-1], gn_mr=sw.mr[j][-1],
                         gn_gamma=gn.weight, gn_beta=gn.bias, act=L.PRO_LRELU, y2=sw.a[j + 1], **gkw)
                if lens is not None:
                    ops.mask_tail(sw.c[j + 1], T, lens)
                    ops.mask_tail(sw.a[j + 1], T, lens)
            inp, T_in = sw.a[-1], T
        self.fwd(self.enc_out, inp, w.z, T_in, bias=self.enc_out.mod.bias, out_f32=True)

    def decoder_fwd(self, w, zq_c, lens=None):
        inp, T_in = zq_c, w.Tz
        for si, st in enumerate(self.dec_stages):
            sw = w.dec[si]
            T, C = sw.T, sw.C
            self.fwd(st.conv, inp, sw.xs[0], T_in, bias=st.conv.mod.bias)
            if lens is not None:
                lens = [n * st.scale for n in lens]
                ops.mask_tail(sw.xs[0], T, lens)
            for j, b in enumerate(st.blocks):
                ci, gn, rs = b.conv_in, b.gn, b.rs
                if lens is not None:
                    self.fwd(ci, sw.xs[j], sw.u[j], T, bias=ci.mod.bias, rowbias=sw.condbias[j])
                    ops.groupnorm_stats_len(sw.u[j], T, 2, lens, w.gn_part, sw.mr[j])
                    ops.gn_glu_fwd_len(sw.u[j], sw.g[j], T, lens, sw.mr[j], gn.weight, gn.bias)
                elif sw.fuse:
                    self.fwd(ci, sw.xs[j], sw.u[j], T, bias=ci.mod.bias, rowbias=sw.condbias[j], gn_stats=w.gst,
                             gn_groups=2)
                    ops.gn_glu_fwd_tiles(sw.u[j], sw.g[j], T, w.gst, sw.mr[j], gn.weight, gn.bias)
                else:
                    self.fwd(ci, sw.xs[j], sw.u[j], T, bias=ci.mod.bias, rowbias=sw.condbias[j])
                    ops.groupnorm_stats(sw.u[j], T, 2, w.gn_part, sw.mr[j])
                    ops.gn_glu_fwd(sw.u[j], sw.g[j], T, sw.mr[j], gn.weight, gn.bias)
                self.fwd(rs, sw.g[j], sw.xs[j + 1], T, bias=rs.mod.bias, res=sw.xs[j], out2=w.skip32, split_col=C,
                         out2_accumulate=(b.gidx > 0))
                if lens is not None:
                    ops.mask_tail(sw.xs[j + 1], T, lens)
            inp, T_in = sw.xs[-1], T
        ops.scale_act_2d(w.skip32, w.a_skip, math.sqrt(1.0 / self.n_dec_layers), L.PRO_RELU)
        self.fwd(self.fin1, w.a_skip, w.f1, w.T, bias=self.fin1.mod.bias, act=L.PRO_RELU)
        self.fwd(self.fin2, w.f1, w.xhat, w.T, bias=self.fin2.mod.bias, out_f32=True)

    def _perm_rows(self, n, K, rank_offset=0, n_local=None):
        perm = torch.randperm(n)[:K]
        if n_local is not None:
            from ..parallel.ddp import owned_rows
            perm = owned_rows(perm, rank_offset, n_local)
        return perm.to(torch.int32)

    def _tile_rows(self, w):
        z = w.z.detach()
        if self.comm is not None:
            z = self.comm.all_gather_cat(z)
        z = z.cpu()
        n, dd = z.shape
        K = self.dims["K"]
        rep = (K + n - 1) // n
        zt = z.repeat(rep, 1)
        zt = zt + torch.randn_like(zt) * (0.01 / np.sqrt(dd))
        rows = zt[torch.randperm(zt.shape[0])][:K]
        return rows.to(self.device, non_blocking=False)

    def jitter_map(self, T):
        p = self.dims["jitter_p"]
        src = np.arange(T, dtype=np.int32)
        cdf0 = np.cumsum([p, 1 - p])
        cdf0 = cdf0 / cdf0[-1]
        rs = np.random.random_sample
        for i in range(T):
            u = rs()
            choice = 1 if u < cdf0[0] else 0
            if choice == 0:
                if i == 0:
                    src[i] = 1
                elif i == T - 1:
                    src[i] = T - 2
                else:
                    u2 = rs()
                    src[i] = i + (-1 if u2 < 0.5 else 1)
        return src

    def _wn_batched(self):
        return self.opt.wn_bwd_batch and self._wn_active

    def _wn_bwd(self, w, key):
        if self._wn_batched():
            self._wn_pending.append(key)
            if self.comm is not None and len(self._wn_pending) >= max(1, self.opt.wn_bwd_ddp_groups):
                self._wn_run(w)
            return
        ops.weight_norm_bwd(w.bwd_tables[key])
        self._grads_final(w.bwd_params[key])

    def _wn_run(self, w):
        keys = tuple(self._wn_pending)
        self._wn_pending = []
        if not keys:
            return
        tab = w.bwd_table_cache.get(keys)
        if tab is None:
            ents = [e for k in keys for e in w.bwd_entries[k]]
            if self.opt.wn_bwd_sort:
                ents.sort(key=_wn_block_bytes, reverse=True)
            tab = w.bwd_table_cache[keys] = ops.wn_table(ents)
            w.bwd_ents_cache[keys] = (ents, ops.weight_norm_bwd_partials(tab))
        if self.comm is None and self.opt.fuse_grad_norm:
            n = w.bwd_ents_cache[keys][1]
            buf = self._sq_buf(w)
            off = self._sq_off
            if off + n > buf.numel():
                raise RuntimeError(f"gradient-norm partials: {off + n} > {buf.numel()}")
            ops.weight_norm_bwd(tab, sq_partials=buf[off:off + n])
            self._sq_off = off + n
            self._sq_runs.append(keys)
        else:
            ops.weight_norm_bwd(tab)
        self._wn_done.update(keys)
        self._grads_final([i for k in keys for i in w.bwd_params[k]])

    def _sq_buf(self, w):
        if getattr(w, "sq_buf", None) is None:
            ents = [e for k in w.bwd_entries for e in w.bwd_entries[k]]
            w.sq_buf = self._zeros(max(1, ops.weight_norm_bwd_partials(ops.wn_table(ents))), dtype=F32)
        return w.sq_buf

    def _sq_finish(self, w):
        runs = tuple(self._sq_runs)
        if not runs:
            return
        plan = w.bwd_sq_cache.get(runs, False)
        if plan is False:
            ents = [e for k in runs for e in w.bwd_ents_cache[k][0]]
            plan = w.bwd_sq_cache[runs] = self._sq_plan(ents, w.sq_buf[:self._sq_off])
        self._sq_plan_ready = plan

    def _sq_plan(self, ents, parts):
        base = self.flat_g.data_ptr()
        iv = []
        for e in ents:
            for k in ("dv", "dg"):
                t = e.get(k)
                if t is None or t.numel() == 0:
                    continue
                lo = (t.data_ptr() - base) // 4
                if not t.is_contiguous() or lo < 0 or lo + t.numel() > self.n_params:
                    return None
                iv.append((lo, lo + t.numel()))
        iv.sort()
        rest, cur = [], 0
        for lo, hi in iv:
            if lo < cur:
                return None
            if lo > cur:
                rest.append((cur, lo - cur))
            cur = hi
        if cur < self.n_params:
            rest.append((cur, self.n_params - cur))
        rng = torch.tensor(rest, dtype=torch.int64).view(-1, 2).to(self.device) if rest else None
        return parts, rng

    def _wn_bwd_flush(self, w):
        if not self._wn_batched():
            return
        done = set(self._wn_pending) | self._wn_done
        if done != set(w.bwd_tables):
            raise RuntimeError(f"batched weight-norm backward: groups {set(w.bwd_tables) - done} did not run")
        self._wn_run(w)

    def _blk(self, w, side, si, j, kind, l):
        parts = w.blk_parts.get((side, si, j))
        return parts[kind][l] if parts is not None else getattr(w, kind)[l]

    def _gnb(self, w, si, j):
        sw = w.enc[si]
        if not sw.fuse:
            return {}
        gn = self.enc_stages[si].blocks[j].gns[-1]
        return dict(gn_bwd=w.gnb_part_enc, gn_h=sw.h[j][-1], gn_mr=sw.mr[j][-1], gn_gamma=gn.weight, gn_beta=gn.bias,
                    gn_groups=1)

    @staticmethod
    def _gnb_parts(sw, cols, fused=True):
        return (sw.T // 128) * ((cols + 127) // 128) if (sw.fuse and fused) else 0

    @staticmethod
    def _bview(buf, B, C):
        return buf.view(-1)[: B * C].view(B, C)

    def _enc_cur(self, w, si, k):
        sw = w.enc[si]
        return Workspace.view(w.dc_flat[k], sw.N, sw.C)

    def _producer_into_enc(self, w, si, dst, colsum_buf, gnb_ok):
        kw = dict(colsum=colsum_buf)
        st = self.enc_stages[si]
        if st.blocks and gnb_ok:
            kw.update(self._gnb(w, si, len(st.blocks) - 1))
        return kw

    def encoder_bwd(self, w, grad_scale=1.0, dz=None):
        B = w.B
        if dz is None and not self.plain:
            ops.vq_commit_bwd_cs(w.z, w.zq, 2.0 * self.m.beta * grad_scale / w.Nz, w.dz, w.cs_eo)
            w.cs_eo_full = True
        else:
            if dz is not None:
                ops.convert_2d(dz, w.dz)
            self.bias_grad(w.cs_eo, w.dz, zero_tail=getattr(w, "cs_eo_full", False))
            w.cs_eo_full = False
        eo = self.enc_out
        ne = len(self.enc_stages)
        last = w.enc[-1]
        k = 0
        cur = self._enc_cur(w, ne - 1, k)
        self.wgrad_dgrad(eo, w.dz, last.a[-1], cur, last.T, mask=last.a[-1], mask_slope=0.2,
                         **self._producer_into_enc(w, ne - 1, None, last.cs[-1], True))
        self._wn_bwd(w, "enc_out")
        for si in reversed(range(ne)):
            st, sw = self.enc_stages[si], w.enc[si]
            T, N, C = sw.T, sw.N, sw.C
            dh = Workspace.view(w.dh_flat, N, C)
            tmp = Workspace.view(w.tmp_flat, N, C)
            dy2 = Workspace.view(w.dy_flat, N, C)
            nb = len(st.blocks)
            top_fused = si == ne - 1 or self.enc_stages[si + 1].conv.kind != KIND_DOWN
            for j in reversed(range(nb)):
                b = st.blocks[j]
                k ^= 1
                nxt = self._enc_cur(w, si, k)
                dy = cur
                fused_here = top_fused if j == nb - 1 else True
                for l in reversed(range(st.L)):
                    Lr, gn = b.convs[l], b.gns[l]
                    cs_b = self._bview(self._blk(w, "enc", si, j, "colsum_b", l), B, C)
                    dg_b = self._bview(self._blk(w, "enc", si, j, "dgam_b", l), B, C)
                    db_b = self._bview(self._blk(w, "enc", si, j, "dbet_b", l), B, C)
                    nparts = self._gnb_parts(sw, C, fused_here) if l == st.L - 1 else 0
                    ops.gn_bwd(dy, sw.h[j][l], dh, T, 1, False, sw.mr[j][l], gn.weight, gn.bias, w.gnb_part_enc,
                               cs_b, dg_b, db_b, nparts=nparts)
                    src = sw.a[j] if l == 0 else sw.g[j][l - 1]
                    if l > 0:
                        self.wgrad_dgrad(Lr, dh, src, dy2, T, mask=sw.g[j][l - 1], mask_slope=0.2)
                        dy = dy2
                    else:
                        self.wgrad_dgrad(Lr, dh, src, tmp, T, mask=sw.a[j], mask_slope=0.2)
                prod = dict(colsum=sw.cs[j])
                if j > 0:
                    prod.update(self._gnb(w, si, j - 1))
                self.wgrad_dgrad(b.skip, cur, sw.c[j], nxt, T, res=tmp, **prod)
                self._wn_bwd(w, b.key)
                cur = nxt
            if si == 0:
                self.wgrad(st.conv, cur, w.x, T)
            else:
                prev = w.enc[si - 1]
                self.wgrad(st.conv, cur, prev.a[-1], T)
                k ^= 1
                pcur = self._enc_cur(w, si - 1, k)
                if st.conv.kind == KIND_DOWN:
                    self.dgrad(st.conv, cur, pcur, T, mask=prev.a[-1], mask_slope=0.2)
                    ops.colsum(pcur, w.cs_part_enc, prev.cs[-1][0])
                else:
                    self.dgrad(st.conv, cur, pcur, T, mask=prev.a[-1], mask_slope=0.2,
                               **self._producer_into_enc(w, si - 1, None, prev.cs[-1], True))
                cur = pcur
            self._wn_bwd(w, ("enc_stage", si))

    def _dec_dr(self, w, si, k):
        return w.dec[si].dr[k]

    def decoder_bwd(self, w):
        B, S = w.B, self.dims["S"]
        f1, f2 = self.fin1, self.fin2
        dxhat = w.dxhat
        ns = len(self.dec_stages)
        self.bias_grad(w.cs_f2, dxhat)
        if self.fin2_pad is not None:
            Fp, wfull = self.fin2_pad
            pol = self.opt.kernel_policy
            ops.conv_dgrad_wgrad(w.dxhat_pad, wfull, w.df1,
                                 dict(T=w.T, cin=Fp, cout=f2.cin, ntaps=1, pad=0, dil=1, policy=pol, mask=w.f1,
                                      mask_slope=0.0, colsum=w.cs_f1),
                                 dxhat, w.f1, f2.slab, dict(T=w.T, ntaps=1, pad=0, dil=1, splits=f2.splits, policy=pol,
                                                            r_dim=f2.cout, c_dim=f2.cin, shift_sign=1))
        else:
            self.wgrad_dgrad(f2, dxhat, w.f1, w.df1, w.T, mask=w.f1, mask_slope=0.0, colsum=w.cs_f1)
        s = math.sqrt(1.0 / self.n_dec_layers)
        lst = ns - 1
        sw = w.dec[lst]
        k = 0
        cur = sw.dr[k]
        self.wgrad_dgrad(f1, w.df1, w.a_skip, cur[:, sw.C:], w.T, mask=w.a_skip, mask_slope=0.0, mask_scale=s,
                         colsum=w.cs_skip)
        targets = [w.dec[si].dr[q][:, w.dec[si].C:] for si in range(ns) if self.dec_stages[si].blocks
                   for q in range(2) if not (si == lst and q == k)]
        if len(targets) == 1:
            ops.convert_2d_zero2(cur[:, sw.C:], targets[0], cur[:, :sw.C])
        else:
            for t in targets:
                ops.convert_2d(cur[:, sw.C:], t)
            ops.convert_2d(None, cur, cols=sw.C)
        self._wn_bwd(w, "fin")
        cur_x = cur[:, :sw.C]
        for si in reversed(range(ns)):
            st, sw = self.dec_stages[si], w.dec[si]
            T, C = sw.T, sw.C
            C2 = 2 * C
            dg = Workspace.view(w.dg_flat, sw.N, C)
            du = Workspace.view(w.du_flat, sw.N, C2)
            for j in reversed(range(len(st.blocks))):
                b = st.blocks[j]
                dg_b = self._bview(self._blk(w, "dec", si, j, "dgam_b", 0), B, C2)
                db_b = self._bview(self._blk(w, "dec", si, j, "dbet_b", 0), B, C2)
                ci, gn, rs = b.conv_in, b.gn, b.rs
                nxt = sw.dr[k ^ 1]
                gkw = dict(gn_bwd=w.gnb_part, gn_h=sw.u[j], gn_mr=sw.mr[j], gn_gamma=gn.weight, gn_beta=gn.bias,
                           gn_groups=2, gn_glu=True) if sw.fuse else {}
                self.wgrad_dgrad(rs, cur, sw.g[j], dg, T, **gkw)
                ops.gn_bwd(dg, sw.u[j], du, T, 2, True, sw.mr[j], gn.weight, gn.bias, w.gnb_part, sw.cs_all[j],
                           dg_b, db_b, nparts=self._gnb_parts(sw, C))
                self.wgrad_dgrad(ci, du, sw.xs[j], nxt[:, :C], T, res=cur[:, :C], colsum=sw.cs[j])
                self._wn_bwd(w, b.key)
                k ^= 1
                cur = nxt
                cur_x = cur[:, :C]
            if st.conv.kind == KIND_UP and not cur_x.is_contiguous():
                ops.convert_2d(cur_x, dg)
                cur_x = dg
            if si > 0:
                prev, pst = w.dec[si - 1], self.dec_stages[si - 1]
                self.wgrad(st.conv, cur_x, prev.xs[-1], T)
                if pst.blocks:
                    k = 0
                    pcur = prev.dr[k]
                    dst = pcur[:, :prev.C]
                else:
                    pcur = None
                    dst = prev.dx
                if st.conv.kind == KIND_UP:
                    self.dgrad(st.conv, cur_x, dst, T)
                    ops.colsum(dst, w.cs_part, prev.cs[-1][0])
                else:
                    self.dgrad(st.conv, cur_x, dst, T, colsum=prev.cs[-1])
                self._wn_bwd(w, ("dec_stage", si))
                cur, cur_x = pcur, dst
            else:
                self.wgrad(st.conv, cur_x, w.zq_in, T)
                if self.plain:
                    self.dgrad(st.conv, cur_x, w.dzq, T)
                self._wn_bwd(w, ("dec_stage", 0))
        emb_g = self.g(self.m.embeds._embedding.weight)
        if not self.cond_groups:
            ops.zero_(emb_g)
        for gi, (O, blocks) in enumerate(self.cond_groups.items()):
            if getattr(w, "cond_ids_mode", False):
                ops.linear_batched_bwd_ids(w.cond_tables[O], self.m.embeds._embedding.weight, w.y_dev, B,
                                           blocks[0].cond.cin, O, w.dyemb, w.lin_part)
            else:
                ops.linear_batched_bwd(w.cond_tables[O], w.yemb, B, blocks[0].cond.cin, O, w.dyemb, w.lin_part)
            ops.embedding_bwd_rows(w.dyemb, w.y_dev, emb_g, accumulate=gi > 0)
        self._wn_bwd_cond(w)

    def _wn_bwd_cond(self, w):
        self._wn_bwd(w, "cond")

    def vq_init_if_needed(self, w):
        q = self.m.quantizer
        if q.initialized:
            return False
        K = self.dims["K"]
        if w.Nz * self.world < K:
            rows = self._tile_rows(w)
            q.embeddings.copy_(rows)
        else:
            perm = self._perm_rows(w.Nz * self.world, K, self.rank * w.Nz, w.Nz if self.comm is not None else None)
            ops.gather_rows_host(w.z, perm, q.embeddings)
            if self.comm is not None:
                self.comm.all_reduce_sum(q.embeddings)
        ops.convert_2d(q.embeddings, q.emb_sum)
        q.emb_elem.fill_(1.0)
        q.mark_initialized()
        return True

    def vq_plain_forward(self, w):
        q = self.m.quantizer
        ops.zero_(w.ema)
        if self.vq_normalize:
            ops.vq_normalize(w.z, q.embeddings.data, w.z_norm, w.z_len, w.embn, w.e_len, w.pv_part, w.stats[2:3])
            zin, emb = w.z_norm, w.embn
        else:
            zin, emb = w.z, q.embeddings.data
        ops.vq_forward(zin, emb, w.idx, w.zq, w.zq_c, w.stats[1:2], w.vq_part, w.bsum, w.bcnt)
        ops.vq_perplexity(w.bcnt, w.Nz, w.stats[4:5])

    def vq_plain_backward(self, w):
        q = self.m.quantizer
        zin = w.z_norm if self.vq_normalize else w.z
        emb = w.embn if self.vq_normalize else q.embeddings.data
        ops.vq_plain_bwd(w.z, zin, w.z_len if self.vq_normalize else None, w.zq, w.dzq,
                         w.src_t if w.jittered else None, w.Tz, self.vq_normalize, float(self.m.beta), 2.0 / w.Nz,
                         w.dz, w.bsum, w.bcnt, emb, w.e_len if self.vq_normalize else None, self.g(q.embeddings))

    def vq_forward_train(self, w, defer_stats=False):
        w.stats_deferred = False
        if self.plain:
            return self.vq_plain_forward(w)
        q = self.m.quantizer
        K = self.dims["K"]
        self.vq_init_if_needed(w)
        w.ev_ema = None
        if self._side_on:
            ops.vq_forward(w.z, q.embeddings, w.idx, w.zq, w.zq_c, w.stats[1:2], w.vq_part, None, None)
            side = self._fork()
            with torch.cuda.stream(side):
                ops.zero_(w.ema)
                ops.vq_stats(w.z, w.idx, K, w.vq_part, w.bsum, w.bcnt)
                self._ema_rows(w, K)
                if self.comm is not None:
                    self.comm.all_reduce_sum(w.ema, async_op=True).wait()
                self._ema_apply(w)
            w.ev_ema = side.record_event()
            return
        if not getattr(w, "ema_clean", False):
            ops.zero_(w.ema)
        w.ema_clean = False
        if defer_stats:
            ops.vq_forward(w.z, q.embeddings, w.idx, w.zq, w.zq_c, None, w.vq_part, None, None)
            w.stats_deferred = True
        else:
            ops.vq_forward(w.z, q.embeddings, w.idx, w.zq, w.zq_c, None, w.vq_part, w.bsum, w.bcnt)
        w.vq_sum_pending = (w.Nz + ops.VQ_FRAMES - 1) // ops.VQ_FRAMES
        self._ema_rows(w, K, defer=self.opt.fused_close and self.comm is None and K <= 512)
        if self.comm is not None:
            self._ema_work = self.comm.all_reduce_sum(w.ema, async_op=True)

    def _ema_rows(self, w, K, defer=False):
        w.ema_perm = None
        if w.Nz * self.world < K:
            rows = self._tile_rows(w)
            if self.rank != 0:
                rows.zero_()
            w.rand_rows.copy_(rows)
        else:
            perm = self._perm_rows(w.Nz * self.world, K, self.rank * w.Nz, w.Nz if self.comm is not None else None)
            if defer:
                w.ema_perm = perm
                return
            ops.gather_rows_host(w.z, perm, w.rand_rows)

    def _ema_apply(self, w, sums=(), publish=None):
        q = self.m.quantizer
        perm = getattr(w, "ema_perm", None)
        res = ops.vq_ema_update(q.emb_sum, q.emb_elem, q.embeddings, w.bsum, w.bcnt, w.rand_rows, q.mu, q.threshold,
                                w.stats[4:8], w.ema_part, clear=True, sums=sums, publish=publish,
                                rows=(w.z, perm) if perm is not None else None)
        w.ema_perm = None
        w.ema_clean = True
        return res

    def vq_ema_update(self, w):
        if self.plain:
            return
        if getattr(w, "ev_ema", None) is not None:
            torch.cuda.current_stream().wait_event(w.ev_ema)
            w.ev_ema = None
            return
        if getattr(w, "ema_applied", False):
            w.ema_applied = False
            return
        self._ema_finish(w)

    def _ema_finish(self, w, sums=(), publish=None):
        if getattr(self, "_ema_work", None) is not None:
            self.comm.wait(self._ema_work, "ema")
# ... 378 lines not shown
```

vae_npvc_amd/ops.py:

```python
import ctypes

import torch

from . import _lib as L
from ._lib import call, ptr, stream_ptr

_DT = {torch.float32: L.VQX_F32, torch.bfloat16: L.VQX_BF16}


def dt_code(dtype: torch.dtype) -> int:
    try:
        return _DT[dtype]
    except KeyError:
        raise L.VqxError(f"unsupported dtype {dtype}") from None


def _check_cuda(*ts):
    for t in ts:
        if t is not None and not t.is_cuda:
            raise L.VqxError("libvqx ops need device tensors (the HIP kernels are the only implementation)")


_debug = False
_logical_end = {}


def set_debug_checks(on):
    global _debug
    prev, _debug = _debug, bool(on)
    return prev


def _span(t, elems, what):
    if not _debug or t is None or elems <= 0:
        return
    st = t.untyped_storage()
    end = _logical_end.get(st.data_ptr(), st.nbytes())
    avail = (end - t.storage_offset() * t.element_size()) // t.element_size()
    if elems > avail:
        raise L.VqxError(f"extent check: {what} needs {elems} elements from its pointer, its buffer holds {avail}")


def _rows(t, rows, ld, cols, what):
    if rows > 0 and t is not None:
        _span(t, (rows - 1) * ld + cols, what)


def _conv_extents(x, w, y, a, bias, rowbias, res, mask, out2, y2, colsum, stats, tiles, gn_h, gn_mr):
    n, cout, cin = a.n_rows, a.cout, a.cin
    split = a.split_col if out2 is not None else 0
    tm = (n + 127) // 128
    _rows(x, n, a.ldx, cin, "conv x")
    _span(w, cout * a.ntaps * cin, "conv w")
    _rows(y, n, a.ldy, split or cout, "conv y")
    _span(bias, cout, "conv bias")
    _span(rowbias, (n // max(1, a.T)) * max(1, a.rowbias_T) * cout, "conv rowbias")
    _rows(res, n, a.ldres, split or cout, "conv res")
    _rows(mask, n, a.ldmask, cout, "conv mask")
    _rows(out2, n, a.ldo2, cout - split, "conv out2")
    _rows(y2, n, a.ldy2, cout, "conv y2")
    _span(colsum, tm * cout, "conv colsum_part")
    _span(stats, (n // 128) * ((cout + 127) // 128) * 4, "conv stat_part")
    _span(tiles, (n // 128) * ((cout + 127) // 128) * 4, "conv gn_stat_tiles")
    _rows(gn_h, n, a.ldgn, cout * (2 if a.gn_glu else 1), "conv gn_h")
    _span(gn_mr, (n // max(1, a.T)) * 2 * max(1, a.gn_groups), "conv gn_mean_rstd")


POLICY_AUTO, POLICY_IM2COL, POLICY_TALL256, POLICY_TALL512, POLICY_TR128, POLICY_K1_2PCU = 0, 1, 2, 3, 4, 5
_policy = POLICY_AUTO


def set_kernel_policy(policy):
    global _policy
    if policy not in (POLICY_AUTO, POLICY_IM2COL, POLICY_TALL256, POLICY_TALL512, POLICY_TR128, POLICY_K1_2PCU):
        raise ValueError(f"kernel policy {policy} not in 0..5")
    prev, _policy = _policy, int(policy)
    return prev


class kernel_policy:

    def __init__(self, policy):
        self.policy = policy

    def __enter__(self):
        self.prev = set_kernel_policy(self.policy)
        return self

    def __exit__(self, *exc):
        set_kernel_policy(self.prev)
        return False


def conv_args(x, w, y, *, T, cin, cout, ntaps, pad, prologue=L.PRO_NONE, pro_scale=1.0, bias=None,
              rowbias=None, res=None, mask=None, mask_slope=0.0, mask_scale=1.0, gn_h=None, gn_mr=None,
              gn_gamma=None, gn_beta=None, out2=None, split_col=0, out2_accumulate=False, out_f32=False,
              act=None, y2=None, colsum=None, gn_stats=None, gn_bwd=None, gn_groups=1, gn_glu=False,
              gn_tiles=None, gn_eps=1e-5, dil=1, policy=None, rowbias_T=0):
    epi = 0
    if bias is not None:
        epi |= L.EPI_BIAS
    if rowbias is not None:
        epi |= L.EPI_ROWBIAS
    if mask is not None:
        epi |= L.EPI_MASK
    if res is not None:
        epi |= L.EPI_RES
    if gn_h is not None and gn_bwd is None:
        epi |= L.EPI_GNADD
    if out2 is not None:
        epi |= L.EPI_SPLIT
    if out_f32:
        epi |= L.EPI_OUTF32
    if act is not None and y2 is None:
        epi |= L.EPI_ACT
    if y2 is not None:
        epi |= L.EPI_ACT2
    if colsum is not None:
        epi |= L.EPI_COLSUM
    if gn_stats is not None:
        epi |= L.EPI_GNSTATS
    if gn_bwd is not None:
        epi |= L.EPI_GNBWD
    a = L.ConvArgs()
    a.x, a.w, a.y = ptr(x), ptr(w), ptr(y)
    a.bias, a.rowbias, a.res, a.mask = ptr(bias), ptr(rowbias), ptr(res), ptr(mask)
    a.gn_h, a.gn_mean_rstd, a.gn_gamma, a.gn_beta, a.out2 = ptr(gn_h), ptr(gn_mr), ptr(gn_gamma), ptr(gn_beta), ptr(out2)
    a.n_rows, a.T, a.cin, a.cout, a.ntaps, a.pad, a.dil = x.shape[0], T, cin, cout, ntaps, pad, dil
    a.kernel_policy = _policy if policy is None else policy
    a.rowbias_T = rowbias_T
    a.ldx, a.ldy = x.stride(0), y.stride(0)
    a.ldres = res.stride(0) if res is not None else 0
    a.ldmask = mask.stride(0) if mask is not None else 0
    a.ldgn = gn_h.stride(0) if gn_h is not None else 0
    a.ldo2 = out2.stride(0) if out2 is not None else 0
    a.dtype = dt_code(x.dtype)
    a.prologue, a.epilogue = prologue, epi
    a.split_col, a.out2_accumulate = split_col, int(bool(out2_accumulate))
    a.pro_scale, a.mask_slope, a.mask_scale = pro_scale, mask_slope, mask_scale
    a.y2, a.ldy2 = ptr(y2), (y2.stride(0) if y2 is not None else 0)
    a.epi_act = act if act is not None else 0
    a.colsum_part = ptr(colsum)
    a.gn_stat_tiles, a.gn_eps = ptr(gn_tiles), gn_eps
    a.stat_part = ptr(gn_stats if gn_stats is not None else gn_bwd)
    a.gn_groups, a.gn_glu = gn_groups, int(gn_glu)
    if _debug:
        _conv_extents(x, w, y, a, bias, rowbias, res, mask, out2, y2, colsum,
                      gn_stats if gn_stats is not None else gn_bwd, gn_tiles, gn_h, gn_mr)
    return a


class LaunchProbe:

    _DT = {L.VQX_F32: "float", L.VQX_BF16: "unsigned short"}

    def __init__(self):
        self.shapes = []

    def clear(self):
        self.shapes = []
        call("vqx_probe_clear")

    def start(self):
        call("vqx_probe_enable", 1)

    def stop(self):
        call("vqx_probe_enable", 0)

    def select(self, info=None):
        if info is None:
            call("vqx_probe_select", None)
        else:
            self._sel = (ctypes.c_int32 * 5)(*info)
            call("vqx_probe_select", self._sel)

    def records(self):
        torch.cuda.synchronize()
        n = ctypes.c_int64()
        call("vqx_probe_count", ctypes.byref(n))
        info = (ctypes.c_int32 * 5)()
        fl, ms = ctypes.c_double(), ctypes.c_float()
        out = []
        for i in range(n.value):
            call("vqx_probe_read", i, info, ctypes.byref(fl), ctypes.byref(ms))
            dt, mode, pro, gen, ek = list(info)
            bk = 64 if dt == L.VQX_BF16 else 32
            if gen == 5:
                sym = {2: f"vqx::dual_tr_kernel<{ek}>", 3: f"vqx::dual_k1_kernel<{ek}>"}.get(pro, "vqx::dual_kernel")
            elif gen == 4:
                sym = f"vqx::conv_gemm3_kernel<{self._DT[dt]}, {mode}, {pro}, false, {ek}>"
            elif gen == 6:
                sym = f"vqx::conv_pp_kernel<{mode}, {ek}, {pro}, 2>"
            elif gen == 2 and mode == 2:
                sym = f"vqx::wgrad_tr_kernel<{ek}, {pro}>"
            elif gen == 3:
                sym = f"vqx::conv_tr8_kernel<{mode}, {ek}, {pro}>"
            elif gen == 2:
                sym = f"vqx::conv_tr_kernel<{mode}, {ek}, {pro}>"
            else:
                sym = f"vqx::conv_gemm_kernel<{self._DT[dt]}, {mode}, {pro}, {'true' if gen else 'false'}, {bk}, 2, {ek}>"
            out.append((sym, fl.value, ms.value * 1e-3, self.shapes[i] if i < len(self.shapes) else "",
                        (dt, mode, pro, gen, ek)))
        return out

    def summary(self, by_shape=False):
        agg = {}
        for key, fl, sec, shape, _ in self.records():
            if by_shape:
                key = f"{key} {shape}"
            a = agg.setdefault(key, [0, 0.0, 0.0])
            a[0] += 1
            a[1] += fl
            a[2] += sec
        return {k: {"launches": n, "flops": f, "seconds": t, "avg_us": 1e6 * t / n, "tflops": f / t / 1e12}
                for k, (n, f, t) in agg.items()}


_probe = None


def set_probe(p):
    global _probe
    if _probe is not None and p is None:
        _probe.stop()
    _probe = p
    if p is not None:
        p.start()


def conv_fwd(x, w, y, **kw):
    _check_cuda(x, w, y)
    a = conv_args(x, w, y, **kw)
    if _probe is not None:
        _probe.shapes.append(f"{a.cin}->{a.cout} k{a.ntaps} epi{a.epilogue}")
    call("vqx_conv1d_fwd", ctypes.byref(a), stream_ptr())
    return y


def conv_dgrad(dy, w, dx, **kw):
    _check_cuda(dy, w, dx)
    a = conv_args(dy, w, dx, **kw)
    if _probe is not None:
        _probe.shapes.append(f"{a.cin}->{a.cout} k{a.ntaps} epi{a.epilogue}")
    call("vqx_conv1d_dgrad", ctypes.byref(a), stream_ptr())
    return dx


def wgrad_args(p, q, slabs, *, T, r_dim, c_dim, ntaps, pad, shift_sign=1, q_prologue=L.PRO_NONE, pro_scale=1.0,
               splits=1, dil=1, policy=None, fixup_dw=None, fixup_counters=None):
    a = L.WgradArgs()
    a.kernel_policy = _policy if policy is None else policy
    a.p, a.q, a.slabs = ptr(p), ptr(q), ptr(slabs)
    a.n_rows, a.T, a.r_dim, a.c_dim, a.ntaps, a.pad, a.shift_sign = p.shape[0], T, r_dim, c_dim, ntaps, pad, shift_sign
    a.ldp, a.ldq = p.stride(0), q.stride(0)
    a.dtype, a.q_prologue, a.splits, a.pro_scale, a.dil = dt_code(p.dtype), q_prologue, splits, pro_scale, dil
    a.slab_dtype = dt_code(slabs.dtype)
    a.fixup_dw, a.fixup_counters = ptr(fixup_dw), ptr(fixup_counters)
    if _debug:
        _span(fixup_dw, r_dim * ntaps * c_dim, "wgrad fixup_dw")
        _rows(p, a.n_rows, a.ldp, r_dim, "wgrad p")
        _rows(q, a.n_rows, a.ldq, c_dim, "wgrad q")
        _span(slabs, splits * r_dim * ntaps * c_dim, "wgrad slabs")
    return a


def conv_wgrad(p, q, slabs, **kw):
    _check_cuda(p, q, slabs)
    a = wgrad_args(p, q, slabs, **kw)
    if _probe is not None:
        _probe.shapes.append(f"{a.r_dim}x{a.ntaps}x{a.c_dim} s{a.splits}")
    call("vqx_conv1d_wgrad", ctypes.byref(a), stream_ptr())
    return slabs


def conv_dgrad_wgrad(dy, w, dx, dgrad_kw, p, q, slabs, wgrad_kw):
    _check_cuda(dy, w, dx, p, q, slabs)
    ad = conv_args(dy, w, dx, **dgrad_kw)
    aw = wgrad_args(p, q, slabs, **wgrad_kw)
    fused = ctypes.c_int32(0)
    call("vqx_conv1d_dgrad_wgrad", ctypes.byref(ad), ctypes.byref(aw), ctypes.byref(fused), stream_ptr())
    if _probe is not None:
        sd = f"{ad.cin}->{ad.cout} k{ad.ntaps} epi{ad.epilogue}"
        sw = f"{aw.r_dim}x{aw.ntaps}x{aw.c_dim} s{aw.splits}"
        _probe.shapes.extend([f"dual {sd} + {sw}"] if fused.value else [sw, sd])
    return bool(fused.value)


def wgrad_tiles(n_rows, T, r_dim, c_dim, ntaps, pad, dtype, q_prologue=L.PRO_NONE, dil=1, policy=POLICY_AUTO):
    t = ctypes.c_int32()
    call("vqx_wgrad_tiles", n_rows, T, r_dim, c_dim, ntaps, pad, dil, dtype, q_prologue, policy, ctypes.byref(t))
    return t.value


def _wn_extents(d):
    kind, cout, cin, k, s = d["kind"], d["cout"], d["cin"], d["k"], d.get("stride", 1) or 1
    if kind == L.WN_COLREDUCE:
        _span(d.get("v"), cin * cout, "colreduce src")
        _span(d.get("dv"), cout, "colreduce dst")
        return
    rows = cin if kind in (1, L.WN_RESAMPLE_T) else cout
    cols = (3 * s * cin if kind == L.WN_RESAMPLE else 3 * s * cout if kind == L.WN_RESAMPLE_T
            else (cout if kind == 1 else cin) * k)
    for key in ("v", "dv"):
        _span(d.get(key), cout * cin * k, f"weight-norm {key}")
    for key in ("g", "dg", "norm"):
        _span(d.get(key), rows, f"weight-norm {key}")
    _span(d.get("w_packed"), rows * cols, "weight-norm w_packed")
    _span(d.get("slabs"), d.get("splits", 1) * rows * cols, "weight-norm slabs")


def wgrad_fixup_ok(n_rows, T, r_dim, c_dim, ntaps, pad, dtype, slab_dtype, q_prologue=L.PRO_NONE, dil=1,
                   policy=POLICY_AUTO):
    ok = ctypes.c_int32()
    call("vqx_wgrad_fixup_ok", n_rows, T, r_dim, c_dim, ntaps, pad, dil, dtype, slab_dtype, q_prologue, policy,
         ctypes.byref(ok))
    return bool(ok.value)


def wn_table(layers):
    arr = (L.WNLayer * len(layers))()
    for i, d in enumerate(layers):
        e = arr[i]
        for k in ("v", "g", "w_packed", "norm", "dv", "dg", "slabs"):
            setattr(e, k, ptr(d.get(k)))
        e.kind, e.cout, e.cin, e.k = d["kind"], d["cout"], d["cin"], d["k"]
        e.splits, e.dtype = d.get("splits", 1), d["dtype"]
        e.stride, e.pad = d.get("stride", 0), d.get("pad", 0)
        sl = d.get("slabs")
        e.slab_dtype = dt_code(sl.dtype) if sl is not None else L.VQX_F32
        if _debug:
            _wn_extents(d)
    raw = bytes(arr)
    dev = torch.frombuffer(bytearray(raw), dtype=torch.uint8).to("cuda")
    return arr, dev


def colreduce_entry(src, dst):
    R, C = src.shape
    return dict(kind=L.WN_COLREDUCE, v=src, dv=dst, cin=R, cout=C, k=1, dtype=L.VQX_F32, splits=1)


def linear_table(layers):
    arr = (L.LinearLayer * len(layers))()
    for i, d in enumerate(layers):
        for k in ("W", "bias", "out", "dout", "dW", "dbias"):
            setattr(arr[i], k, ptr(d.get(k)))
    arr.ents = layers
    dev = torch.frombuffer(bytearray(bytes(arr)), dtype=torch.uint8).to("cuda")
    return arr, dev


def _linear_extents(arr, B, I, O, dc=None, partials=None):
    if not _debug:
        return
    for d in arr.ents:
        _span(d.get("W"), O * I, "linear W")
        _span(d.get("dW"), O * I, "linear dW")
        for key in ("bias", "dbias"):
            _span(d.get(key), O, f"linear {key}")
        for key in ("out", "dout"):
            _span(d.get(key), B * O, f"linear {key}")
    _span(dc, B * I, "linear dc")
    _span(partials, len(arr) * ((O + 63) // 64) * B * I, "linear partials")


def linear_batched_fwd(table, c, B, I, O):
    arr, dev = table
    _linear_extents(arr, B, I, O)
    _span(c, B * I, "linear c")
    call("vqx_linear_batched_fwd", dev.data_ptr(), len(arr), ptr(c), B, I, O, stream_ptr())


def linear_ids_ok(B, I, O, emb):
    return I == 128 and 1 <= B <= 64 and O % 64 == 0 and emb.data_ptr() % 16 == 0


def linear_batched_fwd_ids(table, emb, ids, B, I, O):
    arr, dev = table
    _check_cuda(emb, ids)
    if ids.dtype != torch.int64 or ids.numel() != B:
        raise ValueError("linear_batched_fwd_ids: B int64 ids")
    _linear_extents(arr, B, I, O)
    call("vqx_linear_batched_fwd_ids", dev.data_ptr(), len(arr), ptr(emb), ptr(ids), B, I, O, stream_ptr())


def linear_batched_bwd_ids(table, emb, ids, B, I, O, dc, partials):
    arr, dev = table
    _check_cuda(emb, ids)
    if ids.dtype != torch.int64 or ids.numel() != B:
        raise ValueError("linear_batched_bwd_ids: B int64 ids")
    _linear_extents(arr, B, I, O, dc, partials)
    call("vqx_linear_batched_bwd_ids", dev.data_ptr(), len(arr), ptr(emb), ptr(ids), B, I, O, ptr(dc), ptr(partials),
         stream_ptr())


def linear_batched_bwd(table, c, B, I, O, dc, partials=None):
    arr, dev = table
    if dc is not None and partials is None:
        partials = torch.empty(len(arr) * ((O + 63) // 64) * B * I, device=c.device, dtype=torch.float32)
    _linear_extents(arr, B, I, O, dc, partials)
    _span(c, B * I, "linear c")
    call("vqx_linear_batched_bwd", dev.data_ptr(), len(arr), ptr(c), B, I, O, ptr(dc), ptr(partials), stream_ptr())


WNF_NORMS_READY = 1


def weight_norm_fwd(table, flags=0):
    arr, dev = table
    if flags:
        call("vqx_weight_norm_fwd_flags", ctypes.addressof(arr), dev.data_ptr(), len(arr), flags, stream_ptr())
    else:
        call("vqx_weight_norm_fwd", ctypes.addressof(arr), dev.data_ptr(), len(arr), stream_ptr())


# ... 902 lines not shown
```

Before: 3.646 million mel-frames/s.

## Compute only skip half of last decoder block res/skip conv, fuse skip activation

```diff
diff --git a/include/vqx.h b/include/vqx.h
--- a/include/vqx.h
+++ b/include/vqx.h
@@ -30,7 +30,8 @@
   VQX_EPI_ACT2 = 1 << 8,
   VQX_EPI_COLSUM = 1 << 9,
   VQX_EPI_GNSTATS = 1 << 10,
-  VQX_EPI_GNBWD = 1 << 11
+  VQX_EPI_GNBWD = 1 << 11,
+  VQX_EPI_SPLIT_ACT2 = 1 << 12
 };
 #define VQX_CONV_TILE_ROWS 128
 
@@ -91,6 +92,7 @@
   int32_t kernel_policy;
   float* fixup_dw;
   uint32_t* fixup_counters;
+  int32_t slab_rows;
 } vqx_wgrad_args;
 
 int vqx_conv1d_wgrad(const vqx_wgrad_args* a, vqx_stream_t stream);
@@ -407,6 +409,7 @@
 int vqx_ntc_to_nct_len(const void* y, int32_t ldy, int32_t dtype, int32_t B, int32_t C, int32_t T, const int32_t* len,
                        float* x_nct, int32_t T_out, vqx_stream_t stream);
 
+int vqx_struct_bytes(int32_t* conv_args_bytes, int32_t* wgrad_args_bytes);
 #define VQX_ABI_VERSION 130
 int vqx_version(void);
 
diff --git a/vae_npvc_amd/_lib.py b/vae_npvc_amd/_lib.py
--- a/vae_npvc_amd/_lib.py
+++ b/vae_npvc_amd/_lib.py
@@ -10,7 +10,7 @@
 VQX_F32, VQX_BF16 = 0, 1
 PRO_NONE, PRO_LRELU, PRO_RELU, PRO_SCALE_RELU = 0, 1, 2, 3
 (EPI_BIAS, EPI_ROWBIAS, EPI_MASK, EPI_RES, EPI_GNADD, EPI_SPLIT, EPI_OUTF32, EPI_ACT, EPI_ACT2, EPI_COLSUM, EPI_GNSTATS,
- EPI_GNBWD) = (1 << i for i in range(12))
+ EPI_GNBWD, EPI_SPLIT_ACT2) = (1 << i for i in range(13))
 CONV_TILE_ROWS = 128
 
 c_void_p, c_int32, c_int64, c_float, c_double = (ctypes.c_void_p, ctypes.c_int32, ctypes.c_int64,
@@ -41,6 +41,7 @@
         ("shift_sign", c_int32), ("ldp", c_int32), ("ldq", c_int32), ("dtype", c_int32),
         ("q_prologue", c_int32), ("splits", c_int32), ("pro_scale", c_float), ("dil", c_int32),
         ("slab_dtype", c_int32), ("kernel_policy", c_int32), ("fixup_dw", c_void_p), ("fixup_counters", c_void_p),
+        ("slab_rows", c_int32),
     ]
 
 
@@ -95,6 +96,7 @@
     "vqx_conv1d_wgrad": [ctypes.POINTER(WgradArgs), c_void_p],
     "vqx_conv1d_dgrad_wgrad": [ctypes.POINTER(ConvArgs), ctypes.POINTER(WgradArgs), ctypes.POINTER(ctypes.c_int32),
                                c_void_p],
+    "vqx_struct_bytes": [ctypes.POINTER(c_int32), ctypes.POINTER(c_int32)],
     "vqx_weight_norm_fwd": [c_void_p, c_void_p, c_int32, c_void_p],
     "vqx_weight_norm_bwd": [c_void_p, c_void_p, c_int32, c_void_p],
     "vqx_weight_norm_fwd_flags": [c_void_p, c_void_p, c_int32, c_int32, c_void_p],
@@ -256,6 +258,10 @@
     lib.vqx_version.argtypes = []
     if lib.vqx_version() != ABI_VERSION:
         raise VqxError(f"libvqx ABI {lib.vqx_version()} != expected {ABI_VERSION}; rebuild")
+    nc, nw = c_int32(), c_int32()
+    lib.vqx_struct_bytes(ctypes.byref(nc), ctypes.byref(nw))
+    if (nc.value, nw.value) != (ctypes.sizeof(ConvArgs), ctypes.sizeof(WgradArgs)):
+        raise VqxError("libvqx argument structs differ from this binding's; rebuild")
     _lib = lib
     return lib
 
diff --git a/vae_npvc_amd/csrc/vqx_gemm.hip b/vae_npvc_amd/csrc/vqx_gemm.hip
--- a/vae_npvc_amd/csrc/vqx_gemm.hip
+++ b/vae_npvc_amd/csrc/vqx_gemm.hip
@@ -118,7 +118,12 @@
     }
   }
   if ((epi & VQX_EPI_COLSUM) && !a->colsum_part) { set_error("vqx_conv: COLSUM needs colsum_part [ceil(n_rows/128)][cout]"); return -1; }
-  if (!a->y || !aligned16(a->y)) { set_error("vqx_conv: y must be non-null and 16-byte aligned"); return -1; }
+  if (epi & VQX_EPI_SPLIT_ACT2) {
+    if (mode != MODE_FWD || a->prologue != VQX_PRO_NONE || (epi & ~(VQX_EPI_BIAS | VQX_EPI_SPLIT | VQX_EPI_SPLIT_ACT2)) || !(epi & VQX_EPI_SPLIT)) { set_error("vqx_conv: SPLIT_ACT2 is a forward epilogue with SPLIT, no prologue and no other flag than BIAS"); return -1; }
+    if (a->split_col < 0 || a->split_col >= a->cout) { set_error("vqx_conv: SPLIT_ACT2 needs 0 <= split_col %d < cout %d", a->split_col, a->cout); return -1; }
+    if (!a->y2 || a->ldy2 % 8 || !aligned16(a->y2) || (a->epi_act != VQX_PRO_LRELU && a->epi_act != VQX_PRO_RELU)) { set_error("vqx_conv: SPLIT_ACT2 needs a 16-B aligned y2 with ldy2 %% 8 == 0 and epi_act LRELU or RELU"); return -1; }
+    if (a->y && !aligned16(a->y)) { set_error("vqx_conv: y must be 16-byte aligned"); return -1; }
+  } else if (!a->y || !aligned16(a->y)) { set_error("vqx_conv: y must be non-null and 16-byte aligned"); return -1; }
   if (a->kernel_policy < POL_AUTO || a->kernel_policy > POL_K1_2PCU) { set_error("vqx_conv: kernel_policy %d not in 0..5", a->kernel_policy); return -1; }
 
   P = GemmParams{};
@@ -141,6 +146,16 @@
   P.stat_part = a->stat_part; P.gn_groups = a->gn_groups; P.gn_glu = a->gn_glu;
   P.gn_tiles = a->gn_stat_tiles; P.gn_eps = a->gn_eps;
   P.policy = a->kernel_policy;
+  if (epi & VQX_EPI_SPLIT_ACT2) {
+    const int c0 = a->split_col;
+    P.sel_tiles_n = P.tiles_n;
+    P.b = (const char*)a->w + (int64_t)c0 * a->ntaps * a->cin * es;
+    P.Nc = P.cdim = a->cout - c0;
+    P.b_bytes = (int64_t)a->ntaps * a->cin * P.Nc * es;
+    P.tiles_n = (P.Nc + kBN - 1) / kBN;
+    if (a->bias) P.bias = a->bias + c0;
+    P.split_col = 0;
+  }
   if (a->rowbias_T > 1) {
     const unsigned d = (unsigned)(a->T / a->rowbias_T);
     if ((uint64_t)a->T * d >= (1ull << 32)) { set_error("vqx_conv: rowbias_T: T %d * (T / rowbias_T) must be below 2^32", a->T); return -1; }
@@ -175,6 +190,7 @@
   if (a->n_rows <= 0 || a->T <= 0 || a->n_rows % a->T) { set_error("vqx_conv1d_wgrad: bad n_rows/T"); return -1; }
   if (a->r_dim % epc || a->c_dim % epc || a->ldp % epc || a->ldq % epc || a->c_dim % 8) { set_error("vqx_conv1d_wgrad: dims must be multiples of %d (c_dim of 8)", epc); return -1; }
   if (a->splits < 1) { set_error("vqx_conv1d_wgrad: splits < 1"); return -1; }
+  if (a->slab_rows && a->slab_rows < a->r_dim) { set_error("vqx_conv1d_wgrad: slab_rows %d < r_dim %d", a->slab_rows, a->r_dim); return -1; }
   if (!aligned16(a->p) || !aligned16(a->q) || !a->slabs || !aligned16(a->slabs)) { set_error("vqx_conv1d_wgrad: bad pointers"); return -1; }
   if (a->shift_sign != 1 && a->shift_sign != -1) { set_error("vqx_conv1d_wgrad: shift_sign must be +-1"); return -1; }
   if (a->slab_dtype != VQX_F32 && !(a->slab_dtype == VQX_BF16 && a->dtype == VQX_BF16)) { set_error("vqx_conv1d_wgrad: slab_dtype %d (bf16 slabs need bf16 operands)", a->slab_dtype); return -1; }
@@ -192,12 +208,14 @@
   kps = (kps + kround - 1) / kround * kround;
   P.k_per_split = kps;
   P.y = a->slabs;
+  P.slab_stride = (int64_t)(a->slab_rows ? a->slab_rows : a->r_dim) * P.Nc;
   P.slab_bf16 = a->slab_dtype == VQX_BF16;
   P.policy = a->kernel_policy;
   const int bkv = a->dtype == VQX_BF16 ? 64 : 32;
   gen = (a->T % bkv) != 0 || (a->n_rows % bkv) != 0;
   if (!gen && wgrad_tr_ok(a->n_rows, a->T, a->c_dim, a->ntaps, a->pad, dil, a->dtype == VQX_BF16, a->q_prologue,
                           a->kernel_policy)) {
+    if (a->slab_rows && a->slab_rows != a->r_dim) { set_error("vqx_conv1d_wgrad: slab_rows (a row slice) is not built into the 3-tap tap-reuse kernel"); return -1; }
     P.tap_reuse = 1;
     P.tiles_n = a->c_dim / 64;
   }
@@ -284,6 +302,13 @@
   return 0;
 }
 
+extern "C" int vqx_struct_bytes(int32_t* conv_args_bytes, int32_t* wgrad_args_bytes) {
+  if (!conv_args_bytes || !wgrad_args_bytes) { set_error("vqx_struct_bytes: null"); return -1; }
+  *conv_args_bytes = (int32_t)sizeof(vqx_conv_args);
+  *wgrad_args_bytes = (int32_t)sizeof(vqx_wgrad_args);
+  return 0;
+}
+
 extern "C" int vqx_probe_enable(int32_t on) {
   g_probe_on = on != 0;
   return 0;
diff --git a/vae_npvc_amd/csrc/vqx_gemm_inst.h b/vae_npvc_amd/csrc/vqx_gemm_inst.h
--- a/vae_npvc_amd/csrc/vqx_gemm_inst.h
+++ b/vae_npvc_amd/csrc/vqx_gemm_inst.h
@@ -75,6 +75,7 @@
 }
 
 inline int pick_ek(int epi) {
+  if (epi & VQX_EPI_SPLIT_ACT2) return (epi & ~ek_mask(EK_SPLIT2)) == 0 ? EK_SPLIT2 : EK_ALL;
   for (int ek = EK_NONE; ek < EK_ALL; ++ek)
     if ((epi & ~ek_mask(ek)) == 0) return ek;
   return EK_ALL;
@@ -103,8 +104,9 @@
   const double flops = MODE == MODE_WGRAD ? 2.0 * (double)P.n_rows * P.Mc * P.Nc
                                           : 2.0 * (double)P.n_rows * P.Nc * P.K;
   if constexpr (sizeof(T) == 2 && !GEN && MODE != MODE_WGRAD && PRO == VQX_PRO_NONE &&
-                (EK == EK_NONE || EK == EK_ELEM || EK == EK_SPLIT)) {
-    if (P.ntaps == 1 && three_per_cu(grid, P.policy)) {
+                (EK == EK_NONE || EK == EK_ELEM || EK == EK_SPLIT || EK == EK_SPLIT2)) {
+    const int grid_sel = P.sel_tiles_n ? grid / P.tiles_n * P.sel_tiles_n : grid;
+    if (P.ntaps == 1 && three_per_cu(grid_sel, P.policy)) {
       const int info3[5] = {VQX_BF16, MODE, P.pro, 4, EK};
       gemm_launch((const void*)conv_gemm3_kernel<T, MODE, PRO, GEN, EK>, grid, s, P, info3, flops);
       return;
@@ -171,6 +173,12 @@
       case EK_COLSUM: launch_one<bf16_t, MODE, VQX_PRO_NONE, false, EK_COLSUM>(P, grid, s); break;
       case EK_GNSTATS: launch_one<bf16_t, MODE, VQX_PRO_NONE, false, EK_GNSTATS>(P, grid, s); break;
       case EK_GNBWD: launch_one<bf16_t, MODE, VQX_PRO_NONE, false, EK_GNBWD>(P, grid, s); break;
+      case EK_SPLIT2:
+        if constexpr (MODE == MODE_FWD) {
+          launch_one<bf16_t, MODE, VQX_PRO_NONE, false, EK_SPLIT2>(P, grid, s);
+          break;
+        }
+        [[fallthrough]];
       default: launch_one<bf16_t, MODE, VQX_PRO_NONE, false, EK_ALL>(P, grid, s); break;
     }
   }
diff --git a/vae_npvc_amd/csrc/vqx_gemm_kernel.h b/vae_npvc_amd/csrc/vqx_gemm_kernel.h
--- a/vae_npvc_amd/csrc/vqx_gemm_kernel.h
+++ b/vae_npvc_amd/csrc/vqx_gemm_kernel.h
@@ -66,6 +66,8 @@
   unsigned* fix_cnt;
   int rb_T;
   unsigned rb_magic;
+  int64_t slab_stride;
+  int sel_tiles_n;
 };
 
 template <typename T> struct Cfg;
@@ -197,7 +199,8 @@
   EK_COLSUM = 4,
   EK_GNSTATS = 5,
   EK_GNBWD = 6,
-  EK_ALL = 7
+  EK_ALL = 7,
+  EK_SPLIT2 = 8
 };
 constexpr int kEpiElem = VQX_EPI_BIAS | VQX_EPI_ROWBIAS | VQX_EPI_MASK | VQX_EPI_RES | VQX_EPI_ACT | VQX_EPI_ACT2 |
                          VQX_EPI_OUTF32;
@@ -206,6 +209,7 @@
        : ek == EK_ELEM ? kEpiElem
        : ek == EK_GNADD ? kEpiElem | VQX_EPI_GNADD
        : ek == EK_SPLIT ? kEpiElem | VQX_EPI_SPLIT
+       : ek == EK_SPLIT2 ? kEpiElem | VQX_EPI_SPLIT | VQX_EPI_SPLIT_ACT2
        : ek == EK_COLSUM ? kEpiElem | VQX_EPI_COLSUM
        : ek == EK_GNSTATS ? kEpiElem | VQX_EPI_GNSTATS
        : ek == EK_GNBWD ? kEpiElem | VQX_EPI_COLSUM | VQX_EPI_GNBWD
@@ -354,6 +358,11 @@
       for (int e = 0; e < 8; ++e) v[e] += t[e];
     }
     st8<float>(o2, 0, v);
+    if (epi & VQX_EPI_SPLIT_ACT2) {
+#pragma unroll
+      for (int e = 0; e < 8; ++e) t[e] = apply_pro(P.pro_scale * v[e], P.epi_act, 1.f);
+      st8<T>(P.y2, row * P.ldy2 + (col - P.split_col), t);
+    }
 #pragma unroll
     for (int e = 0; e < 8; ++e) v[e] = 0.f;
     return;
@@ -520,7 +529,8 @@
       const int col = n0 + ec;
       if constexpr (MODE == MODE_WGRAD) {
         if (row < P.Mc && col < P.Nc) {
-          const int64_t at = (int64_t)split * P.Mc * P.Nc + row * P.Nc + col;
+          const int64_t ss = P.slab_stride ? P.slab_stride : (int64_t)P.Mc * P.Nc;
+          const int64_t at = (int64_t)split * ss + row * P.Nc + col;
           if (sizeof(T) == 2 && P.slab_bf16) st8<bf16_t>(P.y, at, v);
           else st8_nt<float, false>((float*)P.y + at, 0, v);
         }
diff --git a/vae_npvc_amd/engine/step.py b/vae_npvc_amd/engine/step.py
--- a/vae_npvc_amd/engine/step.py
+++ b/vae_npvc_amd/engine/step.py
@@ -124,6 +124,14 @@
     side_priority: int = 0
     vq_stats_side: bool = False
     bwd_streams_ddp: bool = True
+    dec_last_skip_only: bool = True
+
+
+def dec_last_block(blocks_per_stage):
+    n = list(blocks_per_stage)
+    if not n or n[-1] <= 0:
+        return None
+    return len(n) - 1, n[-1] - 1
 
 
 class _Stage:
@@ -901,8 +909,27 @@
             inp, T_in = sw.a[-1], T
         self.fwd(self.enc_out, inp, w.z, T_in, bias=self.enc_out.mod.bias, out_f32=True)
 
+    _rs_slab_zero = None
+
+    def _dec_skip_only(self):
+        if not self.opt.dec_last_skip_only:
+            return None
+        at = dec_last_block(len(st.blocks) for st in self.dec_stages)
+        if at is None:
+            return None
+        rs, C = self.dec_stages[at[0]].blocks[at[1]].rs, self.dec_stages[at[0]].C
+        ok = rs.kind == KIND_CONV and rs.k == 1 and rs.cin == C and C % 128 == 0 and (rs.cout - C) % 64 == 0
+        return at if ok and rs.cout > C else None
+
+    def _rs_slab_residual_zero(self, rs, C):
+        if self._rs_slab_zero is not rs.slab or not self.opt.wn_bwd_batch:
+            ops.convert_2d(None, rs.slab.view(rs.splits, -1)[:, :C * rs.cols])
+            self._rs_slab_zero = rs.slab
+
     def decoder_fwd(self, w, zq_c, lens=None):
         inp, T_in = zq_c, w.Tz
+        skip_only = self._dec_skip_only()
+        s_skip = math.sqrt(1.0 / self.n_dec_layers)
         for si, st in enumerate(self.dec_stages):
             sw = w.dec[si]
             T, C = sw.T, sw.C
@@ -924,12 +951,18 @@
                     self.fwd(ci, sw.xs[j], sw.u[j], T, bias=ci.mod.bias, rowbias=sw.condbias[j])
                     ops.groupnorm_stats(sw.u[j], T, 2, w.gn_part, sw.mr[j])
                     ops.gn_glu_fwd(sw.u[j], sw.g[j], T, sw.mr[j], gn.weight, gn.bias)
+                if (si, j) == skip_only:
+                    ops.conv_fwd(sw.g[j], rs.wp, None, T=T, cin=rs.cin, cout=rs.cout, ntaps=1, pad=0, bias=rs.mod.bias,
+                                 out2=w.skip32, split_col=C, out2_accumulate=(b.gidx > 0), out2_act=w.a_skip,
+                                 act=L.PRO_RELU, pro_scale=s_skip, policy=self.opt.kernel_policy)
+                    continue
                 self.fwd(rs, sw.g[j], sw.xs[j + 1], T, bias=rs.mod.bias, res=sw.xs[j], out2=w.skip32, split_col=C,
                          out2_accumulate=(b.gidx > 0))
                 if lens is not None:
                     ops.mask_tail(sw.xs[j + 1], T, lens)
             inp, T_in = sw.xs[-1], T
-        ops.scale_act_2d(w.skip32, w.a_skip, math.sqrt(1.0 / self.n_dec_layers), L.PRO_RELU)
+        if skip_only is None:
+            ops.scale_act_2d(w.skip32, w.a_skip, s_skip, L.PRO_RELU)
         self.fwd(self.fin1, w.a_skip, w.f1, w.T, bias=self.fin1.mod.bias, act=L.PRO_RELU)
         self.fwd(self.fin2, w.f1, w.xhat, w.T, bias=self.fin2.mod.bias, out_f32=True)
 
@@ -1186,7 +1219,11 @@
                          colsum=w.cs_skip)
         targets = [w.dec[si].dr[q][:, w.dec[si].C:] for si in range(ns) if self.dec_stages[si].blocks
                    for q in range(2) if not (si == lst and q == k)]
-        if len(targets) == 1:
+        skip_only = self._dec_skip_only()
+        if skip_only is not None:
+            for t in targets:
+                ops.convert_2d(cur[:, sw.C:], t)
+        elif len(targets) == 1:
             ops.convert_2d_zero2(cur[:, sw.C:], targets[0], cur[:, :sw.C])
         else:
             for t in targets:
@@ -1208,10 +1245,26 @@
                 nxt = sw.dr[k ^ 1]
                 gkw = dict(gn_bwd=w.gnb_part, gn_h=sw.u[j], gn_mr=sw.mr[j], gn_gamma=gn.weight, gn_beta=gn.bias,
                            gn_groups=2, gn_glu=True) if sw.fuse else {}
-                self.wgrad_dgrad(rs, cur, sw.g[j], dg, T, **gkw)
+                last = (si, j) == skip_only
+                if last:
+                    self._rs_slab_residual_zero(rs, C)
+                    pol = self.opt.kernel_policy
+                    dsk = cur[:, C:]
+                    ops.conv_dgrad_wgrad(dsk, rs.wp[C:], dg,
+                                         dict(T=T, cin=rs.cout - C, cout=rs.cin, ntaps=1, pad=0, dil=1, policy=pol, **gkw),
+                                         dsk, sw.g[j], rs.slab[:, C:],
+                                         dict(T=T, ntaps=1, pad=0, dil=1, splits=rs.splits, policy=pol, r_dim=rs.cout - C,
+                                              c_dim=rs.cin, shift_sign=1, slab_rows=rs.cout))
+                else:
+                    if self._rs_slab_zero is rs.slab:
+                        self._rs_slab_zero = None
+                    self.wgrad_dgrad(rs, cur, sw.g[j], dg, T, **gkw)
                 ops.gn_bwd(dg, sw.u[j], du, T, 2, True, sw.mr[j], gn.weight, gn.bias, w.gnb_part, sw.cs_all[j],
                            dg_b, db_b, nparts=self._gnb_parts(sw, C))
-                self.wgrad_dgrad(ci, du, sw.xs[j], nxt[:, :C], T, res=cur[:, :C], colsum=sw.cs[j])
+                if last:
+                    self.wgrad_dgrad(ci, du, sw.xs[j], nxt[:, :C], T, colsum=sw.cs[j])
+                else:
+                    self.wgrad_dgrad(ci, du, sw.xs[j], nxt[:, :C], T, res=cur[:, :C], colsum=sw.cs[j])
                 self._wn_bwd(w, b.key)
                 k ^= 1
                 cur = nxt
diff --git a/vae_npvc_amd/ops.py b/vae_npvc_amd/ops.py
--- a/vae_npvc_amd/ops.py
+++ b/vae_npvc_amd/ops.py
@@ -58,7 +58,7 @@
     _rows(res, n, a.ldres, split or cout, "conv res")
     _rows(mask, n, a.ldmask, cout, "conv mask")
     _rows(out2, n, a.ldo2, cout - split, "conv out2")
-    _rows(y2, n, a.ldy2, cout, "conv y2")
+    _rows(y2, n, a.ldy2, cout - split if a.epilogue & L.EPI_SPLIT_ACT2 else cout, "conv y2")
     _span(colsum, tm * cout, "conv colsum_part")
     _span(stats, (n // 128) * ((cout + 127) // 128) * 4, "conv stat_part")
     _span(tiles, (n // 128) * ((cout + 127) // 128) * 4, "conv gn_stat_tiles")
@@ -96,7 +96,7 @@
               rowbias=None, res=None, mask=None, mask_slope=0.0, mask_scale=1.0, gn_h=None, gn_mr=None,
               gn_gamma=None, gn_beta=None, out2=None, split_col=0, out2_accumulate=False, out_f32=False,
               act=None, y2=None, colsum=None, gn_stats=None, gn_bwd=None, gn_groups=1, gn_glu=False,
-              gn_tiles=None, gn_eps=1e-5, dil=1, policy=None, rowbias_T=0):
+              gn_tiles=None, gn_eps=1e-5, dil=1, policy=None, rowbias_T=0, out2_act=None):
     epi = 0
     if bias is not None:
         epi |= L.EPI_BIAS
@@ -112,10 +112,15 @@
         epi |= L.EPI_SPLIT
     if out_f32:
         epi |= L.EPI_OUTF32
-    if act is not None and y2 is None:
+    if act is not None and y2 is None and out2_act is None:
         epi |= L.EPI_ACT
     if y2 is not None:
         epi |= L.EPI_ACT2
+    if out2_act is not None:
+        if y2 is not None:
+            raise ValueError("conv: out2_act and y2 share the y2 slot")
+        epi |= L.EPI_SPLIT_ACT2
+        y2 = out2_act
     if colsum is not None:
         epi |= L.EPI_COLSUM
     if gn_stats is not None:
@@ -129,7 +134,7 @@
     a.n_rows, a.T, a.cin, a.cout, a.ntaps, a.pad, a.dil = x.shape[0], T, cin, cout, ntaps, pad, dil
     a.kernel_policy = _policy if policy is None else policy
     a.rowbias_T = rowbias_T
-    a.ldx, a.ldy = x.stride(0), y.stride(0)
+    a.ldx, a.ldy = x.stride(0), (y.stride(0) if y is not None else 0)
     a.ldres = res.stride(0) if res is not None else 0
     a.ldmask = mask.stride(0) if mask is not None else 0
     a.ldgn = gn_h.stride(0) if gn_h is not None else 0
@@ -247,7 +252,7 @@
 
 
 def wgrad_args(p, q, slabs, *, T, r_dim, c_dim, ntaps, pad, shift_sign=1, q_prologue=L.PRO_NONE, pro_scale=1.0,
-               splits=1, dil=1, policy=None, fixup_dw=None, fixup_counters=None):
+               splits=1, dil=1, policy=None, fixup_dw=None, fixup_counters=None, slab_rows=0):
     a = L.WgradArgs()
     a.kernel_policy = _policy if policy is None else policy
     a.p, a.q, a.slabs = ptr(p), ptr(q), ptr(slabs)
@@ -256,11 +261,12 @@
     a.dtype, a.q_prologue, a.splits, a.pro_scale, a.dil = dt_code(p.dtype), q_prologue, splits, pro_scale, dil
     a.slab_dtype = dt_code(slabs.dtype)
     a.fixup_dw, a.fixup_counters = ptr(fixup_dw), ptr(fixup_counters)
+    a.slab_rows = slab_rows
     if _debug:
         _span(fixup_dw, r_dim * ntaps * c_dim, "wgrad fixup_dw")
         _rows(p, a.n_rows, a.ldp, r_dim, "wgrad p")
         _rows(q, a.n_rows, a.ldq, c_dim, "wgrad q")
-        _span(slabs, splits * r_dim * ntaps * c_dim, "wgrad slabs")
+        _span(slabs, ((splits - 1) * (slab_rows or r_dim) + r_dim) * ntaps * c_dim, "wgrad slabs")
     return a
 
 
```

Result: no change. 3.668 million mel-frames/s, median of 6 (+0.6%).
